# pairlab/SlotFormer

Hardware: AMD Instinct MI355X
Metric: rollout frames/sec at B=32, 128x128, 7 slots, 6+50 steps (SAVi-encode + SlotFormer rollout) (higher is better)
Workload: dtype f32 storage; matmul/conv on split-bf16 MFMA (bf16x3: hi*hi+hi*lo+lo*hi, f32 accumulate)

## Files before the change

include/slotformer_hip.h:

```cpp
#ifndef SLOTFORMER_HIP_H
#define SLOTFORMER_HIP_H
#include <stddef.h>

#ifdef __cplusplus
extern "C" {
#endif

int sf_version(void);
const char* sf_last_error_string(void);

int sf_get_precision(void);
int sf_set_precision(int mode);

int sf_profile_enable(int class_mask);
int sf_set_seam_fused(int on);
int sf_get_seam_fused(void);
int sf_set_ffn_rows64(int on);
int sf_get_ffn_rows64(void);
int sf_profile_sample(int every);
int sf_profile_read(int kernel_class, double* total_ms, long long* launches, double* work);


int sf_linear_f32(const float* A, int lda, const float* W, const float* bias, const float* ln_gamma,
                  const float* ln_beta, float ln_eps, const float* residual, int ldr, float* C, int ldc,
                  int M, int N, int K, int relu, void* stream);

int sf_layernorm_f32(const float* x, const float* gamma, const float* beta, float* y, int rows, int D,
                     float eps, void* stream);

int sf_conv2d_nchw_in_f32(const float* img, long long frame_stride, const float* weight, const float* bias,
                          const float* add, float* out, int F, int Cin, int Hin, int Win, int Cout, int ks,
                          int stride, int relu, void* stream);
int sf_conv2d_nchw_in_grouped_f32(const float* img, long long frame_stride, int fgroup, long long group_stride, const float* weight,
                                  const float* bias, const float* add, float* out, int F, int Cin, int Hin, int Win, int Cout, int ks,
                                  int stride, int relu, void* stream);

int sf_conv2d_nhwc_f32(const float* in, const float* w_packed, const float* bias, const float* add, float* out,
                       int F, int H, int W, int Cin, int Cout, int ks, int relu, void* stream);
int sf_pack_conv_weight_f32(const float* w_oihw, float* w_ohwi, int Cout, int Cin, int ks, void* stream);
int sf_pixel_feat_f32(const float* x, const float* ln0_g, const float* ln0_b, const float* w1, const float* b1, const float* w2,
                      const float* b2, const float* ln1_g, const float* ln1_b, float* feat, int M, float eps, int form, void* stream);
size_t sf_conv_frag_bytes(int Cout, int Cin, int ks);
int sf_set_conv_fp16x2(int on);
int sf_get_conv_fp16x2(void);
int sf_pack_conv_frag_weights(const float* w_ohwi, void* frag, int Cout, int Cin, int ks, void* stream);
int sf_conv5x5_frag_f32(const float* in, const void* w_frag, const float* bias, const float* add, float* out, int F, int H, int W,
                        int relu, void* stream);
int sf_conv5x5_ws_f32(const float* in, const void* w_frag, const float* bias, const float* add, float* out, int F, int H, int W,
                      int relu, int n_workgroups, void* stream);

size_t sf_deconv_frag_bytes(int Cout, int Cin, int ks, int stride);
int sf_pack_deconv_frag_weights(const float* w_ohwi, void* frag, int Cout, int Cin, int ks, int stride, void* stream);
int sf_deconv5x5s2_frag_f32(const float* in, const void* w_frag, const float* bias, float* out, int R, int H, int W, int relu, void* stream);
int sf_deconv5x5s2_head_frag_f32(const float* in, const void* w_frag, const float* bias, const float* head_w, const float* head_b, float* dec,
                                 int R, int H, int W, void* stream);
int sf_decode_l0_expand_f32(const float* table, const float* posterm, float* out, int R, int res, int C1, void* stream);

int sf_conv_transpose2d_nhwc_f32(const float* in, const float* w_packed, const float* bias, float* out, int F,
                                 int Hin, int Win, int Cin, int Cout, int ks, int stride, int relu, void* stream);
int sf_pack_deconv_weight_f32(const float* w_iohw, float* w_ohwi, int Cin, int Cout, int ks, void* stream);
int sf_slot_broadcast_f32(const float* slots, const float* table, float* out, int R, int P, int D, void* stream);
int sf_decode_combine_f32(const float* dec, float* recon_combined, float* recons, float* masks, int F, int N, int HW,
                          void* stream);
int sf_decode_combine_seg_f32(const float* dec, float* recon_combined, float* recons, float* masks, long long* seg_i64,
                              unsigned char* seg_u8, float fg_thre, unsigned* slot_max, int F, int N, int HW, void* stream);
int sf_postproc_mask_f32(const float* masks, long long* seg_i64, unsigned char* seg_u8, float fg_thre, unsigned* slot_max, int F, int N,
                         int HW, void* stream);

size_t sf_vp_metrics_workspace_bytes(int F, int H, int W);
int sf_vp_image_metrics_f32(const float* gt, const float* pred, double* mse, double* psnr, double* ssim, int F, int H, int W, int to_rgb,
                            void* workspace, size_t workspace_bytes, void* stream);
int sf_vp_mask_metrics(const long long* gt_mask, const void* pred_mask, int pred_is_u8, unsigned* tables, float* pred_boxes, double* ari,
                       double* fari, double* miou, unsigned* flag, int F, int H, int W, int num_classes, void* workspace, size_t workspace_bytes,
                       void* stream);
int sf_vp_bbox_pr_f32(const float* gt_bbox, const unsigned char* gt_pres_mask, const float* pred_bbox, double* ap, double* ar, int F, int N, int M,
                      float ovthresh, void* stream);
int sf_masks_to_boxes(const void* masks, int is_u8, float* boxes, unsigned* flag, int F, int H, int W, int num_boxes, void* stream);
int sf_vp_mean_over_videos_f64(const double* per_video, double* out, int K, int B, int T, void* stream);

typedef struct {
  const void* conv_w[13];
  const float* conv_b[13];
  const float* lin_w[5];
  const float* shift;
  const float* scale;
} sf_lpips_model;
int sf_lpips_pack_conv_weights(const float* w_oihw, void* packed, int Cout, int Cin, void* stream);
int sf_lpips_pack_conv_weights_host(const float* w_oihw, void* packed, int Cout, int Cin);
size_t sf_lpips_workspace_bytes(int H, int W, int chunk);
int sf_lpips_f32(const sf_lpips_model* m, const float* x, const float* y, float* out, int F, int H, int W, int chunk, int normalize,
                 void* workspace, size_t workspace_bytes, void* stream);
int sf_lpips_mean_over_videos_f32(const float* scores, double* per_video, double* mean, int B, int T, void* stream);

size_t sf_ingest_tables_bytes(int H0, int W0, int H, int W, int mode);
int sf_ingest_tables_host(void* tables, size_t bytes, int H0, int W0, int H, int W, int mode);
int sf_ingest_frames_u8(const unsigned char* src, const unsigned char* palette, int K, const void* tables, const float* mean3,
                        const float* std3, float* out, int F, int H0, int W0, int H, int W, int antialias, int max_blocks, void* stream);
int sf_resize_masks_nearest(const void* src, int src_is_u8, const void* tables, long long* out_i64, unsigned char* out_u8, int F, int H0,
                            int W0, int H, int W, void* stream);

int sf_rle_label_maps(const unsigned* run_ends, const int* object_offsets, const int* frame_offsets, const void* tables, long long* labels_i64,
                      unsigned char* labels_u8, int* extents, int F, int num_objects, int num_runs, int h, int w, int H, int W, void* stream);
int sf_rle_boxes_pad(const int* extents, float* bbox, unsigned char* pres_mask, unsigned* flag, int F, int num, void* stream);

enum { SF_EGRESS_TRUNC = 0, SF_EGRESS_NEAREST_EVEN = 1 };
enum { SF_EGRESS_F32_CHW = 0, SF_EGRESS_U8_CHW = 1, SF_EGRESS_U8_HWC = 2 };
enum { SF_EGRESS_IMG = 0, SF_EGRESS_SLOTS = 1, SF_EGRESS_IDS = 2 };
int sf_egress_frames_u8(const float* x, unsigned char* out, long long F, int H, int W, int hwc, int to_rgb, int rounding, void* stream);
typedef struct {
  int kind;
  int N;
  const void* a;
  const void* b;
  float scale;
  int ids_i64;
  int P;
  int history_len;
} sf_egress_tile;
int sf_egress_grid_shape(int K, int H, int W, int nrow, int padding, int border, int* CH, int* CW);
int sf_egress_grid(const sf_egress_tile* tiles, int n_entries, void* out, int out_mode, int T, int H, int W, int nrow, int padding,
                   float pad_value, int border, void* stream);
int sf_egress_draw_boxes(unsigned char* frames, const float* boxes, const unsigned char* pres, const unsigned char* palette, int P, int F, int M,
                         int H, int W, int width, void* stream);

// ... 392 lines not shown
typedef struct {
  int num_slots, slot_size, T, text_len, question_len;
  int d_model, num_heads, ffn_dim, num_layers;
  int vocab, emb_dim;
  int mlp_hidden, num_answers;
  const float* cls;
  const float* pos;
  const float *vision_w, *vision_b;
  const float* q_embedding;
  const float *q_in_proj_w, *q_in_proj_b;
  const sf_tfm_layer* layers;
  const float *cls_w1, *cls_b1, *cls_w2, *cls_b2;
  const float *mc_w1, *mc_b1, *mc_w2, *mc_b2;
} sf_aloe_model;

typedef struct {
  float *cls, *pos, *vision_w, *vision_b, *q_embedding, *q_in_proj_w, *q_in_proj_b;
  const sf_tfm_layer_grads* layers;
  float *cls_w1, *cls_b1, *cls_w2, *cls_b2;
  float *mc_w1, *mc_b1, *mc_w2, *mc_b2;
} sf_aloe_grads;

int sf_aloe_train_ok(int num_slots, int slot_size, int T, int text_len, int d_model, int num_heads, int ffn, int num_layers);
size_t sf_aloe_train_workspace_bytes(const sf_aloe_model* m, int B);
int sf_aloe_train_fwd_f32(const sf_aloe_model* m, const float* slots, long long stride_v, long long stride_t, int V, int T_all, const int* video_index,
                          const int* start, int frame_offset, const int* tokens, const unsigned char* pad_mask, int B1, int Bn, float dropout_p,
                          unsigned long long seed, float* cls_logits, float* mc_logits, unsigned char* gates, unsigned char* head_gates, void* ws,
                          size_t ws_bytes, void* stream);
int sf_aloe_train_bwd_f32(const sf_aloe_model* m, const float* slots, long long stride_v, long long stride_t, int V, int T_all, const int* video_index,
                          const int* start, int frame_offset, const int* tokens, const unsigned char* pad_mask, int B1, int Bn, const float* g_cls,
                          const float* g_mc, const sf_aloe_grads* grads, float dropout_p, unsigned long long seed, void* ws, size_t ws_bytes, void* stream);
int sf_aloe_score_grad_f32(const float* cls_logits, const int* cls_labels, int B1, int num_answers, const float* mc_logits, const float* mc_labels, int Bn,
                           float w_cls, float w_mc, float* losses, float* g_cls, float* g_mc, void* stream);

int sf_rollout_train_clips_fwd_f32(const sf_rollouter* m, const float* table, int T_total, const int* clip_video, const int* clip_start,
                                   int frame_offset, float* pred, int B, int pred_len, float dropout_p, unsigned long long seed, void* ws,
                                   size_t ws_bytes, void* stream);
size_t sf_clip_mse_workspace_bytes(int B, int S, long long E);
int sf_clip_mse_f32(const float* pred, const float* target, const int* clip_video, const int* clip_start, int T_total, int first_frame,
                    int frame_step, const float* step_w, const int* clip_len, int hist, float scale, float* d_pred, double* stats, int B, int S,
                    long long E, void* ws, size_t ws_bytes, void* stream);
int sf_clip_frames_f32(const unsigned char* table, int T_total, const int* clip_video, const int* clip_start, int first_frame, int frame_step,
                       const float* mean3, const float* std3, float* out, int B, int S, int H, int W, void* stream);

int sf_normal_noise_f32(float* out, long long n, unsigned long long seed, unsigned tag, void* stream);
size_t sf_kernel_sample_workspace_bytes(long long R, int D);
int sf_kernel_sample_fwd_f32(const float* dist, const float* noise, unsigned long long seed, unsigned tag, float prior_log_var, float* kernels,
                             double* kld_sum, long long R, int D, void* ws, size_t ws_bytes, void* stream);
int sf_kernel_sample_bwd_f32(const float* dist, const float* noise, unsigned long long seed, unsigned tag, float prior_log_var,
                             const float* d_kernels, const float* d_kld, float kld_scale, float* d_dist, long long R, int D, void* stream);

typedef struct {
  int resolution;
  int enc_layers;
  int enc_channels[9];
  int enc_ks;
  int enc_out_channels, num_slots, slot_size, slot_mlp_size, num_iterations;
  const float* conv_w[8];
  const float* conv_b[8];
  const float* pos_table;
  const float *enc_ln_g, *enc_ln_b, *enc_fc1_w, *enc_fc1_b, *enc_fc2_w, *enc_fc2_b;
  const float *sa_norm_in_g, *sa_norm_in_b, *sa_q_ln_g, *sa_q_ln_b, *sa_q_w;
  const float* sa_kv_w;
  const float *gru_w_ih, *gru_w_hh, *gru_b_ih, *gru_b_hh;
  const float *mlp_ln_g, *mlp_ln_b, *mlp_w1, *mlp_b1, *mlp_w2, *mlp_b2;
  const float* init_latents;
  int kd_mode;
  const float *kd_w0, *kd_b0, *kd_ln_g, *kd_ln_b, *kd_w3, *kd_b3;
  int pred_type;
  int pred_rnn, pred_norm_first, pred_num_layers, pred_num_heads, pred_ffn_dim, pred_hidden;
  const float *pm_ln_g, *pm_ln_b, *pm_w0, *pm_b0, *pm_w2, *pm_b2;
  const sf_tfm_layer* pred_layers;
  const float *lstm_w_ih, *lstm_w_hh, *lstm_b_ih, *lstm_b_hh, *proj_w, *proj_b;
  float sa_eps;
  const float* sa_q_w_t;
  const float *pm_w0_t, *pm_w2_t, *kd_w0_t;
  const void *sa_gru_ih_p, *sa_gru_hh_p, *sa_mlp_w1_p, *sa_mlp_w2_p, *sa_q_w_p;
  const float *sa_fold_q_w, *sa_fold_q_w_t, *sa_fold_gru_ih_t;
  const void *sa_fold_q_w_p, *sa_fold_gru_ih_p;
  const void** pred_packed;
  const void *enc_fc1_p, *enc_fc2_p;
  const void* conv_w_frag[8];
  const void *pm_w0_p, *pm_w2_p, *kd_w0_p;
} sf_savi_encoder;

size_t sf_savi_encode_workspace_bytes(const sf_savi_encoder* m, int B);
int sf_savi_encode_f32(const sf_savi_encoder* m, const float* img, const float* noise, const float* prev_slots,
                       float* lstm_h, float* lstm_c, int state_valid, float* post_slots, float* kernel_dist,
                       float* attn, int B, int T, void* ws, size_t ws_bytes, void* stream);

size_t sf_savi_cnn_workspace_bytes(const sf_savi_encoder* m, int B);
int sf_savi_cnn_f32(const sf_savi_encoder* m, const float* img, int B, int T, int t0, int t1, float* feat, void* ws,
                    size_t ws_bytes, void* stream);
int sf_savi_encode_pre_f32(const sf_savi_encoder* m, const float* img, const float* feat_pre, int n_pre, const float* noise,
                           const float* prev_slots, float* lstm_h, float* lstm_c, int state_valid, float* post_slots,
                           float* kernel_dist, float* attn, int B, int T, void* ws, size_t ws_bytes, void* stream);
size_t sf_savi_encode_fork_workspace_bytes(const sf_savi_encoder* m, int B, int T);
size_t sf_savi_encode_batched_workspace_bytes(const sf_savi_encoder* m, int B, int T);
int sf_set_encode_fuse_next(int on);
int sf_get_encode_fuse_next(void);
int sf_set_slot_chain(int on);
int sf_get_slot_chain(void);
int sf_set_slot_attn_planes(int on);
int sf_get_slot_attn_planes(void);
int sf_set_pixel_tok(int on);
int sf_get_pixel_tok(void);
int sf_savi_chain_ok(const sf_savi_encoder* m, int B, int T);
size_t sf_savi_planes_bytes(const sf_savi_encoder* m, int B, int T);
size_t sf_savi_features_workspace_bytes(const sf_savi_encoder* m, int B, int T);
int sf_savi_features_planes_f32(const sf_savi_encoder* m, const float* img, int B, int T, void* planes, void* ws, size_t ws_bytes, void* stream);
size_t sf_savi_slots_chain_workspace_bytes(const sf_savi_encoder* m, int videos);
int sf_savi_slots_chain_f32(const sf_savi_encoder* m, const void* planes, const float* noise, const float* prev_slots, float* post, long long post_bs,
                            float* kernel_dist, float* attn, int NB, int B, int T, void* ws, size_t ws_bytes, void* stream);
int sf_savi_encode_fork_f32(const sf_savi_encoder* m, const float* img, const float* feat_pre, int n_pre, const float* noise,
                            const float* prev_slots, float* lstm_h, float* lstm_c, int state_valid, float* post_slots,
                            float* kernel_dist, float* attn, int B, int T, void* ws, size_t ws_bytes, void* stream, void* side_stream);

typedef struct {
  int resolution;
  int dec_layers;
  int dec_channels[9];
  int dec_strides[8];
  int dec_ks, dec_res;
  int num_slots, slot_size;
  const float* deconv_w[8];
  const float* deconv_b[8];
  const float *out_w, *out_b;
  const float* pos_table;
  const float* deconv_w_flipped[8];
  const void* deconv_w_frag[8];
  const float* l0_weff;
  const float* l0_posterm;
} sf_savi_decoder;

size_t sf_savi_decode_workspace_bytes(const sf_savi_decoder* m, int F);
int sf_savi_decode_f32(const sf_savi_decoder* m, const float* slots, float* recon_combined, float* recons,
                       float* masks, int F, void* ws, size_t ws_bytes, void* stream);
int sf_savi_decode_seg_f32(const sf_savi_decoder* m, const float* slots, float* recon_combined, float* recons, float* masks,
                           long long* seg_i64, unsigned char* seg_u8, float fg_thre, int F, void* ws, size_t ws_bytes, void* stream);

typedef struct {
  float* deconv_w[8];
  float* deconv_b[8];
  float *out_w, *out_b, *pos_w, *pos_b;
} sf_savi_decoder_grads;

size_t sf_savi_decode_train_workspace_bytes(const sf_savi_decoder* m, int F);
int sf_savi_decode_train_fwd_f32(const sf_savi_decoder* m, const float* slots, float* recon_combined, float* recons,
                                 float* masks, int F, void* ws, size_t ws_bytes, void* stream);
int sf_savi_decode_train_bwd_f32(const sf_savi_decoder* m, const float* const* deconv_w_bwd, const float* d_recon,
                                 float* d_slots, const float* pos_grid, const sf_savi_decoder_grads* g, int F, void* ws,
                                 size_t ws_bytes, void* stream);

size_t sf_conv_wgrad_partial_floats(int CA, int ks);
int sf_conv_wgrad_f32(const float* A, int CA, int F, int H, int W, const float* X, int Hx, int Wx, int s, int ks, long long rows, float* dW,
                      float* partial, size_t partial_floats, void* stream);
int sf_conv2d_nhwc_bwd_data_f32(const float* in, const float* w_packed, const float* relu_mask, float* out, int F, int Hin, int Win, int Cin,
                                int Cout, int ks, int stride, void* stream);
int sf_pack_conv_bwd_weight_f32(const float* w_oihw, float* w_bwd, int Cout, int Cin, int ks, void* stream);
size_t sf_conv_first_wgrad_workspace_bytes(int F);
int sf_conv_first_wgrad_f32(const float* img, long long frame_stride, int resolution, const float* dY, int F, float* dW, void* ws,
                            size_t ws_bytes, void* stream);
int sf_pos_dense_grad_f32(const float* d, int F, int HW, int C, const float* grid, float* dw, float* db, float* dtab, void* stream);
size_t sf_savi_decode_head_bwd_workspace_bytes(int Cl);
int sf_savi_decode_head_bwd_f32(const float* dec, const float* d_recon, const float* act, const float* out_w, float* d_dec, float* d_act,
                                float* d_out_w, float* d_out_b, int F, int N, int HW, int Cl, void* ws, size_t ws_bytes, void* stream);
// ... 51 lines not shown
```

slotformer_amd/_lib.py:

```python
import ctypes as C
import os

_HERE = os.path.dirname(os.path.abspath(__file__))
LIB_PATH = os.environ.get('SF_LIB_PATH') or os.path.join(_HERE, 'libslotformer_hip.so')

FP = C.c_void_p


class sf_tfm_layer(C.Structure):
    _fields_ = [(n, FP) for n in (
        'norm1_g', 'norm1_b', 'in_proj_w', 'in_proj_b', 'out_proj_w', 'out_proj_b',
        'norm2_g', 'norm2_b', 'lin1_w', 'lin1_b', 'lin2_w', 'lin2_b', 'lin1_packed', 'lin2_packed', 'attn_in_packed', 'attn_out_packed', 'tok_packed')]


class sf_rollouter(C.Structure):
    _fields_ = [(n, C.c_int) for n in (
        'num_slots', 'slot_size', 'd_model', 'num_layers', 'num_heads', 'ffn_dim', 'norm_first',
        'window_len', 'single_step')] + [(n, FP) for n in (
            'in_proj_w', 'in_proj_b', 'out_proj_w', 'out_proj_b', 'pe_tok')] + [
                ('layers', C.POINTER(sf_tfm_layer)), ('in_proj_packed', C.c_void_p), ('out_proj_packed', C.c_void_p)]


class sf_aloe(C.Structure):
    _fields_ = [(n, C.c_int) for n in ('num_slots', 'slot_size', 'T', 'text_len', 'question_len', 'd_model', 'num_heads', 'ffn_dim', 'num_layers',
# ... 16 lines not shown
        (n, FP) for n in ('in_proj_w', 'in_proj_b', 'enc_t_pe', 'cls')] + [('layers', C.POINTER(sf_tfm_layer))] + [
            (n, FP) for n in ('mlp_w1', 'mlp_b1', 'mlp_w2', 'mlp_b2')]


class sf_phyre_readout_grads(C.Structure):
    _fields_ = [(n, FP) for n in ('in_proj_w', 'in_proj_b', 'enc_t_pe', 'cls')] + [('layers', C.POINTER(sf_tfm_layer_grads))] + [
        (n, FP) for n in ('mlp_w1', 'mlp_b1', 'mlp_w2', 'mlp_b2')]


_ALOE_HEADS = ('cls_w1', 'cls_b1', 'cls_w2', 'cls_b2', 'mc_w1', 'mc_b1', 'mc_w2', 'mc_b2')
_ALOE_LEAVES = ('cls', 'pos', 'vision_w', 'vision_b', 'q_embedding', 'q_in_proj_w', 'q_in_proj_b')


class sf_aloe_model(C.Structure):
    _fields_ = [(n, C.c_int) for n in ('num_slots', 'slot_size', 'T', 'text_len', 'question_len', 'd_model', 'num_heads', 'ffn_dim', 'num_layers',
                                       'vocab', 'emb_dim', 'mlp_hidden', 'num_answers')] + [(n, FP) for n in _ALOE_LEAVES] + [
                                           ('layers', C.POINTER(sf_tfm_layer))] + [(n, FP) for n in _ALOE_HEADS]


class sf_aloe_grads(C.Structure):
    _fields_ = [(n, FP) for n in _ALOE_LEAVES] + [('layers', C.POINTER(sf_tfm_layer_grads))] + [(n, FP) for n in _ALOE_HEADS]


class sf_rollouter_grads(C.Structure):
    _fields_ = [(n, FP) for n in ('in_proj_w', 'in_proj_b', 'out_proj_w', 'out_proj_b')] + [
        ('layers', C.POINTER(sf_tfm_layer_grads)), ('pe_tok', FP)]


_SA_LEAVES = ('norm_in_g', 'norm_in_b', 'wk', 'wv', 'q_ln_g', 'q_ln_b', 'wq', 'gru_w_ih', 'gru_w_hh', 'gru_b_ih', 'gru_b_hh',
              'mlp_ln_g', 'mlp_ln_b', 'mlp_w1', 'mlp_b1', 'mlp_w2', 'mlp_b2')


class sf_slot_attention(C.Structure):
    _fields_ = [(n, C.c_int) for n in ('in_features', 'slot_size', 'mlp_hidden', 'num_slots')] + [
        (n, FP) for n in _SA_LEAVES] + [('eps', C.c_float)]


class sf_slot_attention_grads(C.Structure):
    _fields_ = [(n, FP) for n in _SA_LEAVES]


class sf_adam_group(C.Structure):
    _fields_ = [('begin', C.c_longlong), ('lr', C.c_float)]


class sf_savi_decoder_grads(C.Structure):
    _fields_ = [('deconv_w', FP * 8), ('deconv_b', FP * 8)] + [(n, FP) for n in ('out_w', 'out_b', 'pos_w', 'pos_b')]


class sf_savi_features(C.Structure):
    _fields_ = [(n, C.c_int) for n in ('resolution', 'layers', 'channels', 'ks', 'hidden', 'out_channels')] + [
        ('conv_w', FP * 8), ('conv_b', FP * 8)] + [(n, FP) for n in ('pos_grid', 'pos_w', 'pos_b', 'ln_g', 'ln_b', 'fc1_w', 'fc1_b',
                                                                      'fc2_w', 'fc2_b')]


class sf_savi_features_grads(C.Structure):
    _fields_ = [('conv_w', FP * 8), ('conv_b', FP * 8)] + [(n, FP) for n in ('pos_w', 'pos_b', 'ln_g', 'ln_b', 'fc1_w', 'fc1_b',
                                                                              'fc2_w', 'fc2_b')]


class sf_savi_encoder(C.Structure):
    _fields_ = (
        [('resolution', C.c_int), ('enc_layers', C.c_int), ('enc_channels', C.c_int * 9),
         ('enc_ks', C.c_int)] +
        [(n, C.c_int) for n in ('enc_out_channels', 'num_slots', 'slot_size', 'slot_mlp_size',
                                'num_iterations')] +
        [('conv_w', FP * 8), ('conv_b', FP * 8), ('pos_table', FP)] +
        [(n, FP) for n in ('enc_ln_g', 'enc_ln_b', 'enc_fc1_w', 'enc_fc1_b', 'enc_fc2_w', 'enc_fc2_b',
                           'sa_norm_in_g', 'sa_norm_in_b', 'sa_q_ln_g', 'sa_q_ln_b', 'sa_q_w', 'sa_kv_w',
                           'gru_w_ih', 'gru_w_hh', 'gru_b_ih', 'gru_b_hh',
                           'mlp_ln_g', 'mlp_ln_b', 'mlp_w1', 'mlp_b1', 'mlp_w2', 'mlp_b2',
                           'init_latents')] +
        [('kd_mode', C.c_int)] +
        [(n, FP) for n in ('kd_w0', 'kd_b0', 'kd_ln_g', 'kd_ln_b', 'kd_w3', 'kd_b3')] +
        [(n, C.c_int) for n in ('pred_type', 'pred_rnn', 'pred_norm_first', 'pred_num_layers',
                                'pred_num_heads', 'pred_ffn_dim', 'pred_hidden')] +
        [(n, FP) for n in ('pm_ln_g', 'pm_ln_b', 'pm_w0', 'pm_b0', 'pm_w2', 'pm_b2')] +
        [('pred_layers', C.POINTER(sf_tfm_layer))] +
        [(n, FP) for n in ('lstm_w_ih', 'lstm_w_hh', 'lstm_b_ih', 'lstm_b_hh', 'proj_w', 'proj_b')] +
        [('sa_eps', C.c_float), ('sa_q_w_t', FP), ('pm_w0_t', FP), ('pm_w2_t', FP), ('kd_w0_t', FP),
         ('sa_gru_ih_p', C.c_void_p), ('sa_gru_hh_p', C.c_void_p), ('sa_mlp_w1_p', C.c_void_p), ('sa_mlp_w2_p', C.c_void_p),
         ('sa_q_w_p', C.c_void_p), ('sa_fold_q_w', FP), ('sa_fold_q_w_t', FP), ('sa_fold_gru_ih_t', FP), ('sa_fold_q_w_p', C.c_void_p),
         ('sa_fold_gru_ih_p', C.c_void_p), ('pred_packed', C.POINTER(C.c_void_p)), ('enc_fc1_p', C.c_void_p), ('enc_fc2_p', C.c_void_p),
         ('conv_w_frag', C.c_void_p * 8), ('pm_w0_p', C.c_void_p), ('pm_w2_p', C.c_void_p), ('kd_w0_p', C.c_void_p)])


class sf_slate_block(C.Structure):
    _fields_ = [(n, FP) for n in ('ln1_g', 'ln1_b', 'wqkv', 'wo', 'ln2_g', 'ln2_b', 'wq_c', 'wkv_c', 'wo_c', 'ln3_g', 'ln3_b',
                                  'w1', 'b1', 'w2', 'b2')] + [('is_first', C.c_int)]


class sf_slate_decoder(C.Structure):
    _fields_ = [(n, C.c_int) for n in ('d_model', 'num_heads', 'num_layers', 'vocab_size', 'num_slots', 'max_len')] + [
        (n, FP) for n in ('in_proj_w', 'in_proj_b', 'tok_emb', 'pos_emb', 'lnf_g', 'lnf_b', 'head_w')] + [
            ('blocks', C.POINTER(sf_slate_block))]


class sf_slate_step_opts(C.Structure):
    _fields_ = [('soft_rows', FP), ('conv0_t', FP), ('conv0_width', C.c_int), ('soft_scale', C.c_float), ('soft_seed', C.c_ulonglong),
                ('sample', C.c_int), ('inv_temperature', C.c_float), ('sample_seed', C.c_ulonglong), ('row_base', C.c_longlong)]


class sf_savi_decoder(C.Structure):
    _fields_ = ([('resolution', C.c_int), ('dec_layers', C.c_int), ('dec_channels', C.c_int * 9),
                 ('dec_strides', C.c_int * 8), ('dec_ks', C.c_int), ('dec_res', C.c_int), ('num_slots', C.c_int),
                 ('slot_size', C.c_int), ('deconv_w', FP * 8), ('deconv_b', FP * 8), ('out_w', FP), ('out_b', FP),
                 ('pos_table', FP), ('deconv_w_flipped', FP * 8), ('deconv_w_frag', C.c_void_p * 8), ('l0_weff', FP), ('l0_posterm', FP)])


class sf_egress_tile(C.Structure):
    _fields_ = [('kind', C.c_int), ('N', C.c_int), ('a', C.c_void_p), ('b', C.c_void_p), ('scale', C.c_float), ('ids_i64', C.c_int), ('P', C.c_int),
                ('history_len', C.c_int)]


class sf_lpips_model(C.Structure):
    _fields_ = [('conv_w', C.c_void_p * 13), ('conv_b', FP * 13), ('lin_w', FP * 5), ('shift', FP), ('scale', FP)]


I, LL, F32, SZ, VP = C.c_int, C.c_longlong, C.c_float, C.c_size_t, C.c_void_p

SIGNATURES = {
    'sf_version': (I, []),
    'sf_last_error_string': (C.c_char_p, []),
    'sf_get_precision': (I, []),
    'sf_set_precision': (I, [I]),
    'sf_profile_enable': (I, [I]),
    'sf_profile_sample': (I, [I]),
    'sf_set_seam_fused': (I, [I]),
    'sf_get_seam_fused': (I, []),
    'sf_set_ffn_rows64': (I, [I]),
    'sf_get_ffn_rows64': (I, []),
    'sf_profile_read': (I, [I, C.POINTER(C.c_double), C.POINTER(C.c_longlong), C.POINTER(C.c_double)]),
    'sf_linear_f32': (I, [FP, I, FP, FP, FP, FP, F32, FP, I, FP, I, I, I, I, I, VP]),
    'sf_layernorm_f32': (I, [FP, FP, FP, FP, I, I, F32, VP]),
    'sf_conv2d_nchw_in_f32': (I, [FP, LL, FP, FP, FP, FP, I, I, I, I, I, I, I, I, VP]),
    'sf_conv2d_nchw_in_grouped_f32': (I, [FP, LL, I, LL, FP, FP, FP, FP, I, I, I, I, I, I, I, I, VP]),
    'sf_conv2d_nhwc_f32': (I, [FP, FP, FP, FP, FP, I, I, I, I, I, I, I, VP]),
    'sf_pack_conv_weight_f32': (I, [FP, FP, I, I, I, VP]),
    'sf_pixel_feat_f32': (I, [FP] * 10 + [I, F32, I, VP]),
    'sf_conv_frag_bytes': (SZ, [I, I, I]),
    'sf_set_conv_fp16x2': (I, [I]),
    'sf_get_conv_fp16x2': (I, []),
    'sf_pack_conv_frag_weights': (I, [FP, VP, I, I, I, VP]),
    'sf_conv5x5_frag_f32': (I, [FP, VP, FP, FP, FP, I, I, I, I, VP]),
    'sf_conv5x5_ws_f32': (I, [FP, VP, FP, FP, FP, I, I, I, I, I, VP]),
    'sf_deconv_frag_bytes': (SZ, [I, I, I, I]),
    'sf_pack_deconv_frag_weights': (I, [FP, VP, I, I, I, I, VP]),
    'sf_deconv5x5s2_frag_f32': (I, [FP, VP, FP, FP, I, I, I, I, VP]),
    'sf_deconv5x5s2_head_frag_f32': (I, [FP, VP, FP, FP, FP, FP, I, I, I, VP]),
    'sf_decode_l0_expand_f32': (I, [FP, FP, FP, I, I, I, VP]),
    'sf_conv_transpose2d_nhwc_f32': (I, [FP, FP, FP, FP, I, I, I, I, I, I, I, I, VP]),
    'sf_pack_deconv_weight_f32': (I, [FP, FP, I, I, I, VP]),
    'sf_slot_broadcast_f32': (I, [FP, FP, FP, I, I, I, VP]),
    'sf_decode_combine_f32': (I, [FP, FP, FP, FP, I, I, I, VP]),
    'sf_savi_decode_workspace_bytes': (SZ, [C.POINTER(sf_savi_decoder), I]),
    'sf_savi_decode_f32': (I, [C.POINTER(sf_savi_decoder), FP, FP, FP, FP, I, VP, SZ, VP]),
    'sf_savi_decode_seg_f32': (I, [C.POINTER(sf_savi_decoder), FP, FP, FP, FP, VP, VP, F32, I, VP, SZ, VP]),
    'sf_decode_combine_seg_f32': (I, [FP, FP, FP, FP, VP, VP, F32, VP, I, I, I, VP]),
    'sf_postproc_mask_f32': (I, [FP, VP, VP, F32, VP, I, I, I, VP]),
    'sf_vp_metrics_workspace_bytes': (SZ, [I, I, I]),
    'sf_vp_image_metrics_f32': (I, [FP, FP, VP, VP, VP, I, I, I, I, VP, SZ, VP]),
    'sf_vp_mask_metrics': (I, [VP, VP, I, VP, FP, VP, VP, VP, VP, I, I, I, I, VP, SZ, VP]),
    'sf_vp_bbox_pr_f32': (I, [FP, VP, FP, VP, VP, I, I, I, F32, VP]),
    'sf_masks_to_boxes': (I, [VP, I, FP, VP, I, I, I, I, VP]),
    'sf_vp_mean_over_videos_f64': (I, [VP, VP, I, I, I, VP]),
    'sf_lpips_pack_conv_weights': (I, [FP, VP, I, I, VP]),
    'sf_lpips_pack_conv_weights_host': (I, [VP, VP, I, I]),
    'sf_lpips_workspace_bytes': (SZ, [I, I, I]),
    'sf_lpips_f32': (I, [C.POINTER(sf_lpips_model), FP, FP, FP, I, I, I, I, I, VP, SZ, VP]),
    'sf_lpips_mean_over_videos_f32': (I, [FP, VP, VP, I, I, VP]),
    'sf_ingest_tables_bytes': (SZ, [I, I, I, I, I]),
    'sf_ingest_tables_host': (I, [VP, SZ, I, I, I, I, I]),
    'sf_ingest_frames_u8': (I, [VP, VP, I, VP, FP, FP, FP, I, I, I, I, I, I, I, VP]),
    'sf_resize_masks_nearest': (I, [VP, I, VP, VP, VP, I, I, I, I, I, VP]),
    'sf_rle_label_maps': (I, [VP, VP, VP, VP, VP, VP, VP, I, I, I, I, I, I, I, VP]),
    'sf_rle_boxes_pad': (I, [VP, FP, VP, VP, I, I, VP]),
    'sf_egress_frames_u8': (I, [FP, VP, LL, I, I, I, I, I, VP]),
    'sf_egress_grid_shape': (I, [I, I, I, I, I, I, C.POINTER(I), C.POINTER(I)]),
    'sf_egress_grid': (I, [C.POINTER(sf_egress_tile), I, VP, I, I, I, I, I, I, F32, I, VP]),
    'sf_egress_draw_boxes': (I, [VP, FP, VP, VP, I, I, I, I, I, I, VP]),
    'sf_pos_embed_table_f32': (I, [FP, FP, FP, FP, I, I, VP]),
    'sf_slot_attn_num_partials': (I, [I]),
    'sf_slot_attn_iter_f32': (I, [FP, FP, I, LL, FP, FP, FP, FP, I, I, I, I, F32, F32, VP]),
    'sf_slot_update_f32': (I, [FP, FP, I, FP] + [FP] * 10 + [FP, I, I, I, I, F32, VP]),
    'sf_slot_update_packed_f32': (I, [FP, FP, I, FP, VP, VP, FP, FP, FP, FP, VP, FP, VP, FP, FP, FP, FP, VP, FP, I, I, I, I, F32, VP]),
    'sf_slot_attn_iter_planes_f32': (I, [VP, LL, FP, FP, FP, FP, LL, I, I, I, F32, F32, VP]),
    'sf_slot_prologue_f32': (I, [FP] * 8 + [I, FP, FP, FP, LL, FP, LL, FP, FP, FP, FP, FP, I, I, I, F32, VP]),
    'sf_slot_update_packed_next_f32': (I, [FP, FP, I, FP, VP, VP, FP, FP, FP, FP, VP, FP, VP, FP, FP, FP, FP, VP, FP, I, I, I, I, F32,
                                           FP, LL, I, FP, FP, VP, FP, VP, FP, I, VP, FP, FP, LL, FP, LL, FP, VP]),
    'sf_mha_f32': (I, [FP, FP, I, I, I, I, I, VP]),
    'sf_qkv_attention_f32': (I, [FP, FP, FP, F32, FP, FP, FP, I, I, I, I, I, VP]),
    'sf_lstm_pointwise_f32': (I, [FP, FP, FP, FP, I, I, VP]),
    'sf_sample_dist_f32': (I, [FP, FP, FP, I, I, VP]),
    'sf_bilinear_resize_f32': (I, [FP, FP, LL, I, I, I, I, VP]),
    'sf_rollout_workspace_bytes': (SZ, [C.POINTER(sf_rollouter), I]),
    'sf_rollout_f32': (I, [C.POINTER(sf_rollouter), FP, I, I, I, VP, SZ, VP]),
    'sf_rollout_opts_f32': (I, [C.POINTER(sf_rollouter), FP, I, I, I, VP, SZ, VP, C.POINTER(sf_rollout_opts)]),
    'sf_rollout_phases_workspace_bytes': (SZ, [C.POINTER(sf_rollouter), I, I]),
    'sf_rollout_phases_f32': (I, [C.POINTER(sf_rollouter), FP, I, I, I, I, I, VP, SZ, VP, C.POINTER(sf_rollout_opts)]),
    'sf_rollout_uses_seam': (I, [C.POINTER(sf_rollouter), I]),
    'sf_rollout_uses_seam_opts': (I, [C.POINTER(sf_rollouter), I, C.POINTER(sf_rollout_opts)]),
    'sf_rollout_is_fused': (I, [C.POINTER(sf_rollouter)]),
    'sf_rollout_tok_ok': (I, [C.POINTER(sf_rollouter)]),
    'sf_rollout_tok_layers': (I, [C.POINTER(sf_rollouter), I, C.POINTER(sf_rollout_opts)]),
    'sf_ffn_chunk_partials_f32': (I, [C.POINTER(sf_tfm_layer), FP, LL, FP, LL, I, I, I, VP]),
    'sf_attn_block_f32': (I, [C.POINTER(sf_tfm_layer), FP, FP, I, I, I, I, VP]),
    'sf_ffn_block_rows_f32': (I, [C.POINTER(sf_tfm_layer), FP, FP, I, I, VP]),
    'sf_set_layer_tok': (I, [I]),
    'sf_get_layer_tok': (I, []),
    'sf_layer_tok_packed_bytes': (SZ, []),
    'sf_layer_tok_packed_bytes_ex': (SZ, [I, I, I]),
    'sf_pack_layer_tok_weights': (I, [C.POINTER(sf_tfm_layer), VP, I, I, I, VP]),
    'sf_layer_tok_block_f32': (I, [C.POINTER(sf_tfm_layer), I, FP, FP, I, I, VP]),
    'sf_layer_tok_block_ex_f32': (I, [C.POINTER(sf_tfm_layer), I, I, I, I, FP, FP, I, I, VP]),
    'sf_debug_read_ts_layer_tok': (I, [C.POINTER(C.c_longlong)]),
    'sf_attn_rows_planes_bytes': (SZ, [I]),
    'sf_attn_block_rows_f32': (I, [C.POINTER(sf_tfm_layer), FP, FP, VP, I, I, I, VP]),
    'sf_slot_attn_iter_bwd_workspace_bytes': (SZ, [I, I, I, I]),
    'sf_slot_attn_iter_bwd_f32': (I, [FP, FP, I, LL, FP, FP, FP, I, FP, FP, FP, I, FP, I, I, I, I, F32, F32, VP, SZ, VP]),
    'sf_slot_attn_iter_bwd16_workspace_bytes': (SZ, [I, I, I, I]),
    'sf_slot_attn_iter_bwd16_f32': (I, [FP, FP, I, LL, FP, FP, FP, I, FP, FP, FP, I, FP, I, I, I, I, F32, F32, VP, SZ, VP]),
    'sf_set_slot_attn_tile16': (I, [I]),
# ... 268 lines not shown
```

slotformer_amd/csrc/engine.hip:

```cpp
#include "../../include/slotformer_hip.h"
#include "sf_internal.h"
#include "sf_arena.h"
#include <map>
#include <vector>
#include "layer_fused.h"
#include "slot_chain.h"
#include <stdlib.h>

namespace {

inline bool plain_gemms(const SfThreadOpts& o) { return o.precision == 2 || o.precision == 3; }

struct TfmWs {
  float *x2, *qkv, *att, *hid, *y;
};

bool tfm_ws_take(SfArena& bp, TfmWs& w, int M, int d, int ffn) {
  w.x2 = bp.take((size_t)M * d);
  w.qkv = bp.take((size_t)M * 3 * d);
  w.att = bp.take((size_t)M * d);
  w.hid = bp.take((size_t)M * ffn);
  w.y = bp.take((size_t)M * d);
  return bp.ok;
}
// ... 434 lines not shown
}

size_t sf_rollout_phases_workspace_bytes(const sf_rollouter* m, int B, int frame_offset) {
  if (!m || B <= 0 || frame_offset <= 0 || (long long)B * frame_offset > 0x7fffffffLL) return 0;
  return sf_rollout_workspace_bytes(m, B * frame_offset);
}

int sf_rollout_phases_f32(const sf_rollouter* m, float* slots, int B, int T_total, int obs, int frame_offset, int pred_len, void* ws,
                          size_t ws_bytes, void* stream, const sf_rollout_opts* opts) {
  SF_REQUIRE(m && slots && ws, "null pointer");
  SF_REQUIRE(B >= 1 && pred_len >= 0, "bad batch / pred_len");
  SF_REQUIRE(frame_offset >= 1, "sf_rollout_phases_f32: frame_offset >= 1");
  SF_REQUIRE(!(m->single_step && frame_offset > 1), "sf_rollout_phases_f32: a single-step rollouter takes frame_offset 1 only");
  SF_REQUIRE(m->window_len >= 1, "bad rollouter shape");
  const int f = frame_offset, hist = m->single_step ? 1 : m->window_len;
  SF_REQUIRE((long long)obs >= (long long)hist * f, "sf_rollout_phases_f32: fewer observed frames than burn-in * frame_offset");
  const long long S = ((long long)pred_len + f - 1) / f;
  SF_REQUIRE((long long)T_total >= obs + S * f, "slots buffer shorter than obs + ceil(pred_len / frame_offset) * frame_offset");
  const int first = obs - hist * f;
  if (!opts) return rollout_run(m, slots, B, T_total, first, f, (int)S, ws, ws_bytes, stream);
  SF_TRY(check_rollout_opts(opts));
  OptsScope scope(rollout_thread_opts(opts));
  return rollout_run(m, slots, B, T_total, first, f, (int)S, ws, ws_bytes, stream);
}

int sf_rollout_is_fused(const sf_rollouter* m) { return plan_rollout(m, 1, sf_thread_opts()).fused(); }

int sf_rollout_tok_ok(const sf_rollouter* m) {
  SfThreadOpts o = sf_thread_opts();
  o.layer_tok = 1;
  const RolloutPlan p = plan_rollout(m, 1, o);
  return p.fused() && p.tok_layers > 0;
}

int sf_rollout_tok_layers(const sf_rollouter* m, int B, const sf_rollout_opts* opts) {
  if (B <= 0) return 0;
  return plan_rollout(m, B, rollout_thread_opts(opts)).tok_layers;
}

int sf_rollout_uses_seam_opts(const sf_rollouter* m, int B, const sf_rollout_opts* opts) {
  if (B <= 0 || !plan_rollout(m, B, rollout_thread_opts(opts)).seam) return 0;
  for (int s = 1; s <= m->window_len; ++s) {
    int nf, f0;
    step_window(m, s, nf, f0);
    if (sf_seam_window_ok(nf * m->num_slots, m->num_slots)) return 1;
  }
  return 0;
}
int sf_rollout_uses_seam(const sf_rollouter* m, int B) { return sf_rollout_uses_seam_opts(m, B, nullptr); }

int sf_rollout_bf16(const sf_rollouter* m, float* slots, int B, int T_total, int pred_len, void* ws, size_t ws_bytes,
                    void* stream) {
  sf_rollout_opts o = {2, -1, 0, 0};
  return sf_rollout_opts_f32(m, slots, B, T_total, pred_len, ws, ws_bytes, stream, &o);
}

}

namespace {
int enc_chunk(int B) { return B < 32 ? B : 32; }
constexpr int ENC_FORK_AHEAD = 4;
int enc_fork_steps(int T) { return T < 2 ? 2 : (T < ENC_FORK_AHEAD ? T : ENC_FORK_AHEAD); }
constexpr int ENC_HW = 64 * 64;

int enc_cmax(const sf_savi_encoder* m) {
  int cmax = 0;
  for (int i = 1; i <= m->enc_layers && i < 9; ++i) cmax = m->enc_channels[i] > cmax ? m->enc_channels[i] : cmax;
  return cmax;
}
void enc_cnn_take(SfArena& bp, float** buf, int n, const sf_savi_encoder* m, size_t frames) {
  for (int i = 0; i < n; ++i) buf[i] = bp.take(frames * ENC_HW * enc_cmax(m));
}

struct SlotRows { float *a, *b, *lat, *q; };
void slot_rows_take(SfArena& bp, SlotRows& r, size_t rows, int D) {
  for (float** f : {&r.a, &r.b, &r.lat, &r.q}) *f = bp.take(rows * D);
}

struct EncodePlan {
  bool fork = false;
  int KV = 2;
  int n_pre = 0;
  bool batched = false;
  enum Feat { KV_GEMMS, KV_FUSED, FOLD_ROWS, FOLD_192, FOLD_PLANES } feat = KV_GEMMS;
  const float *q_w = nullptr, *q_w_t = nullptr, *gru_ih_t = nullptr;
  const void *q_w_p = nullptr, *gru_ih_p = nullptr;
  enum Update { VALU, WIDE, MFMA } update = VALU;
  int p_step = 1;
  bool pred_step = false;
  bool prologue = false;
  bool fuse_next = false;
  bool chain_model = false;
  bool chain = false;
  bool fold() const { return feat >= FOLD_ROWS; }
};

struct EncodeWs {
  float* feat[2];
  float *h1, *h2;
  float* kv;
  SlotRows rows;
  float *lnbuf, *px;
  float *kdist, *kdtmp;
  float *pnum, *pden;
  TfmWs tw;
  float* gates;
  float* big[3];
  float* planes;
};

bool enc_ws_take(SfArena& bp, EncodeWs& w, const sf_savi_encoder* m, int B, int T, const EncodePlan& p) {
  const int N = m->num_slots, D = m->slot_size, Ce = m->enc_out_channels, P = sf_sa_pick_partials(ENC_HW);
  const size_t R = (size_t)B * N, Bc = enc_chunk(B), HW = ENC_HW;
  enc_cnn_take(bp, w.feat, 2, m, Bc);
  w.h1 = bp.take(Bc * HW * Ce);
  w.h2 = bp.take(Bc * HW * Ce);
  w.kv = bp.take((size_t)p.KV * B * HW * 2 * D);
  slot_rows_take(bp, w.rows, R, D);
  w.lnbuf = bp.take(R * D);
  w.px = bp.take(R * D);
  w.kdist = bp.take(R * 2 * D);
  w.kdtmp = bp.take(R * 2 * D);
  w.pnum = bp.take((size_t)B * P * N * D);
  w.pden = bp.take((size_t)B * P * N);
  tfm_ws_take(bp, w.tw, (int)R, D, m->pred_ffn_dim > 2 * D ? m->pred_ffn_dim : 2 * D);
  w.gates = bp.take(R * 4 * (m->pred_hidden > 0 ? m->pred_hidden : 1));
  if (p.batched) enc_cnn_take(bp, w.big, 3, m, (size_t)B * T);
  if (p.chain) w.planes = bp.take((size_t)B * T * HW * 128);
  return bp.ok;
}

size_t enc_ws_bytes(const sf_savi_encoder* m, int B, int T, const EncodePlan& p) {
  SfArena bp(nullptr);
  EncodeWs w;
  enc_ws_take(bp, w, m, B, T, p);
  return bp.bytes() + 8192;
}

bool enc_batched_ok(const sf_savi_encoder* m, int B, int T, int precision) {
  if (T < 2 || B > enc_chunk(B) || (long long)B * T > 384 || m->enc_layers < 2 || precision != 1) return false;
  for (int i = 1; i < m->enc_layers; ++i)
    if (!m->conv_w_frag[i] || m->enc_channels[i] != 64 || m->enc_channels[i + 1] != 64) return false;
  return true;
}

EncodePlan plan_encode(const sf_savi_encoder* m, int B, int T, int n_pre, bool fork, size_t ws_bytes) {
  EncodePlan p;
  p.fork = fork;
  p.KV = fork ? enc_fork_steps(T) : 2;
  p.n_pre = n_pre;
  if (!m || m->enc_layers < 1 || m->enc_layers > 8) return p;
  const int precision = sf_get_precision();
  const int HW = ENC_HW, N = m->num_slots, D = m->slot_size, Ce = m->enc_out_channels, Hm = m->slot_mlp_size, P = sf_sa_pick_partials(HW);
  const int Cl = m->enc_channels[m->enc_layers];
  const bool feat192 = Cl == 64 && Ce == 192 && m->enc_fc1_p && m->enc_fc2_p;
  const bool fold = precision >= 1 && m->sa_fold_q_w && m->sa_fold_q_w_t && m->sa_fold_gru_ih_t && Ce == D && (sf_pixel_mlp_feat_ok(Cl, Ce) || feat192);
  const bool planes = fold && !feat192 && sf_switch(SF_SW_SLOT_ATTN_PLANES) && sf_slot_attn_planes_ok(HW, D, N) && Cl == 64 && P == HW / 256;
  p.feat = fold ? (feat192 ? EncodePlan::FOLD_192 : planes ? EncodePlan::FOLD_PLANES : EncodePlan::FOLD_ROWS)
                : (precision >= 1 ? EncodePlan::KV_FUSED : EncodePlan::KV_GEMMS);
  p.q_w = fold ? m->sa_fold_q_w : m->sa_q_w;
  p.q_w_t = fold ? m->sa_fold_q_w_t : m->sa_q_w_t;
  p.gru_ih_t = fold ? m->sa_fold_gru_ih_t : m->gru_w_ih;
  p.q_w_p = fold ? m->sa_fold_q_w_p : m->sa_q_w_p;
  p.gru_ih_p = fold ? m->sa_fold_gru_ih_p : m->sa_gru_ih_p;
  const bool su_packed = precision >= 1 && p.gru_ih_p && m->sa_gru_hh_p && m->sa_mlp_w1_p && m->sa_mlp_w2_p && p.q_w_p;
  p.update = !su_packed ? EncodePlan::VALU : sf_slot_update_mfma_ok(D, Hm, P) ? EncodePlan::MFMA
            : sf_slot_update_wide_ok(D, Hm, P) ? EncodePlan::WIDE : EncodePlan::VALU;
  if (fold && P == HW / 256 && (planes || sf_slot_attn_sparse_records_n(nullptr, nullptr, HW, D, N))) p.p_step = 2;
  p.pred_step = m->pred_type == 1 && m->pred_packed && precision >= 1;
  p.prologue = m->pred_type == 0 && !m->pred_rnn && m->kd_mode == 1 && m->pm_w0_t && m->pm_w2_t && m->kd_w0_t && p.q_w_t;
  p.fuse_next = p.prologue && p.update == EncodePlan::MFMA && m->pm_w0_p && m->pm_w2_p && m->kd_w0_p && m->pm_ln_g && m->pm_ln_b && m->pm_b0 &&
                m->pm_b2 && m->kd_b0 && sf_switch(SF_SW_ENCODE_FUSE_NEXT);
  p.chain_model = precision == 1 && fold && p.feat != EncodePlan::FOLD_192 && p.update == EncodePlan::MFMA && p.fuse_next &&
                  sf_slot_chain_ok(D, Hm, HW, N) && m->init_latents && m->enc_fc1_w && m->enc_fc2_w;
  p.batched = !fork && n_pre == 0 && enc_batched_ok(m, B, T, precision);
  p.chain = p.batched && p.chain_model && sf_switch(SF_SW_SLOT_CHAIN);
  if (p.chain && ws_bytes < enc_ws_bytes(m, B, T, p)) p.chain = false;
  if (p.batched && ws_bytes < enc_ws_bytes(m, B, T, p)) p.batched = false;
  return p;
}

int run_cnn_layers(const sf_savi_encoder* m, const float* src, long long frame_stride, int nb, float* dst, float* featA, float* featB,
                   int i0, int i1, hipStream_t st) {
  const int res = m->resolution;
  for (int i = i0; i < i1; ++i) {
    const bool lastc = (i == m->enc_layers - 1);
    const int cin = m->enc_channels[i], cout = m->enc_channels[i + 1];
    const float* add = lastc ? m->pos_table : nullptr;
    float* out = lastc ? dst : ((i & 1) ? featB : featA);
    const float* cur = i == 0 ? nullptr : (((i - 1) & 1) ? featB : featA);
    if (i == 0) {
      SF_TRY(sf_conv2d_nchw_in_f32(src, frame_stride, m->conv_w[0], m->conv_b[0], add, out, nb, cin, res, res, cout,
                                   m->enc_ks, res == 128 ? 2 : 1, lastc ? 0 : 1, st));
    } else {
      int rc = 1;
      if (rc == 1 && m->conv_w_frag[i])
        rc = sf_conv5x5_ws_ex(cur, m->conv_w_frag[i], m->conv_b[i], add, out, nb, 64, 64, cin, cout, m->enc_ks, lastc ? 0 : 1, 0, st);
      if (rc == 1 && m->conv_w_frag[i])
        rc = sf_conv5x5_rows4_ex(cur, m->conv_w_frag[i], m->conv_b[i], add, out, nb, 64, 64, cin, cout, m->enc_ks, lastc ? 0 : 1, st);
      if (rc < 0 || rc > 1) return rc;
      if (rc == 1)
        SF_TRY(sf_conv2d_nhwc_f32(cur, m->conv_w[i], m->conv_b[i], add, out, nb, 64, 64, cin, cout, m->enc_ks, lastc ? 0 : 1, st));
    }
  }
  return 0;
}

int enc_cnn_all_steps(const sf_savi_encoder* m, const float* img, int B, int T, float* const* big, hipStream_t st) {
  const int res = m->resolution, c1 = m->enc_channels[1];
  const long long frame_elems = (long long)3 * res * res;
  const int rc = sf_conv_first_grouped_ex(img, (long long)T * frame_elems, B, frame_elems, m->conv_w[0], m->conv_b[0], nullptr, big[0], B * T,
                                          m->enc_channels[0], res, res, c1, m->enc_ks, res == 128 ? 2 : 1, 1, st);
  if (rc < 0 || rc > 1) return rc;
  for (int t = 0; t < T && rc == 1; ++t)
    SF_TRY(sf_conv2d_nchw_in_f32(img + (long long)t * frame_elems, (long long)T * frame_elems, m->conv_w[0], m->conv_b[0], nullptr,
                                 big[0] + (long long)t * B * ENC_HW * c1, B, m->enc_channels[0], res, res, c1, m->enc_ks, res == 128 ? 2 : 1, 1, st));
  return run_cnn_layers(m, nullptr, 0, B * T, big[2], big[0], big[1], 1, m->enc_layers, st);
}

int enc_feature_planes(const sf_savi_encoder* m, const float* img, int B, int T, float* const* big, void* planes, hipStream_t st) {
  SF_TRY(enc_cnn_all_steps(m, img, B, T, big, st));
  return sf_pixel_mlp_feat_planes_ex(big[2], m->enc_ln_g, m->enc_ln_b, m->enc_fc1_w, m->enc_fc1_b, m->enc_fc2_w, m->enc_fc2_b, m->sa_norm_in_g, m->sa_norm_in_b,
                                     planes, B * T * ENC_HW, 1e-5f, st);
}
int enc_slots_chain(const sf_savi_encoder* m, const void* planes, const float* noise, const float* prev, float* post, long long post_bs, float* kernel_dist,
                    float* attn, int NB, int B, int T, const SlotRows& r, hipStream_t st) {
  const int N = m->num_slots, D = m->slot_size;
  const float ln_eps = 1e-5f;
  const int pr = sf_slot_prologue_ex(prev, m->init_latents, m->pm_ln_g, m->pm_ln_b, m->pm_w0_t, m->pm_b0, m->pm_w2_t, m->pm_b2, m->pred_norm_first, m->kd_w0_t,
                                     m->kd_b0, noise, (long long)T * N * D, kernel_dist, (long long)T * N * 2 * D, m->sa_q_ln_g, m->sa_q_ln_b, m->sa_fold_q_w_t,
                                     r.a, r.q, NB * B, N, D, ln_eps, st);
  if (pr != 0) return pr < 0 ? pr : sf_set_err(-1, "the one-launch slot prologue does not apply to this model", __FILE__, __LINE__);
  SfChainWeights cw;
  cw.gru_ih_p = m->sa_fold_gru_ih_p; cw.gru_hh_p = m->sa_gru_hh_p; cw.gru_b_ih = m->gru_b_ih; cw.gru_b_hh = m->gru_b_hh; cw.ln_g = m->mlp_ln_g; cw.ln_b = m->mlp_ln_b;
  cw.w1_p = m->sa_mlp_w1_p; cw.b1 = m->mlp_b1; cw.w2_p = m->sa_mlp_w2_p; cw.b2 = m->mlp_b2; cw.q_ln_g = m->sa_q_ln_g; cw.q_ln_b = m->sa_q_ln_b; cw.q_w_p = m->sa_fold_q_w_p;
  cw.pm_ln_g = m->pm_ln_g; cw.pm_ln_b = m->pm_ln_b; cw.pm_w0_p = m->pm_w0_p; cw.pm_b0 = m->pm_b0; cw.pm_w2_p = m->pm_w2_p; cw.pm_b2 = m->pm_b2;
  cw.pm_norm_first = m->pred_norm_first; cw.kd_w_p = m->kd_w0_p; cw.kd_b = m->kd_b0;
  return sf_slot_chain_ex(planes, NB, B, T, ENC_HW, N, m->num_iterations, 1.0f / sqrtf((float)D), m->sa_eps, ln_eps, r.a, r.b, r.lat, r.q, post, post_bs, attn,
                          noise, kernel_dist, &cw, st);
}

hipEvent_t enc_fork_event(int i) {
  thread_local std::map<int, std::vector<hipEvent_t>> per_dev;
  int dev = 0;
  if (hipGetDevice(&dev) != hipSuccess) return nullptr;
  std::vector<hipEvent_t>& ev = per_dev[dev];
  while ((int)ev.size() <= i) {
    hipEvent_t e = nullptr;
    if (hipEventCreateWithFlags(&e, hipEventDisableTiming) != hipSuccess) return nullptr;
    ev.push_back(e);
  }
  return ev[i];
}
int enc_fork_record(int i, hipStream_t s) {
  const hipEvent_t e = enc_fork_event(i);
  SF_REQUIRE(e != nullptr, "hipEventCreate failed");
  return hipEventRecord(e, s) == hipSuccess ? 0 : sf_set_err((int)hipGetLastError(), "hipEventRecord", __FILE__, __LINE__);
}
int enc_fork_wait(int i, hipStream_t s) {
  return hipStreamWaitEvent(s, enc_fork_event(i), 0) == hipSuccess ? 0 : sf_set_err((int)hipGetLastError(), "hipStreamWaitEvent", __FILE__, __LINE__);
}

struct EncodeArgs {
  const sf_savi_encoder* m;
  const float *img, *feat_pre, *noise;
  float *lstm_h, *lstm_c, *post, *kernel_dist, *attn;
  int B, T;
};

int enc_step_features(const EncodeArgs& a, const EncodePlan& p, const EncodeWs& w, int t, float* kv, hipStream_t st) {
  const sf_savi_encoder* m = a.m;
  const int HW = ENC_HW, B = a.B, Bc = enc_chunk(B), Cl = m->enc_channels[m->enc_layers], Ce = m->enc_out_channels, D = m->slot_size;
  const long long frame_elems = (long long)3 * m->resolution * m->resolution;
  const float ln_eps = 1e-5f;
  for (int b0 = 0; b0 < B; b0 += Bc) {
    const int nb = (B - b0 < Bc) ? (B - b0) : Bc, Mp = nb * HW;
    const float* cur;
    if (t < p.n_pre) {
      cur = a.feat_pre + ((long long)t * B + b0) * HW * Cl;
    } else if (p.batched) {
      cur = w.big[2] + ((long long)t * B + b0) * HW * Cl;
    } else {
      float* dstf = (m->enc_layers & 1) ? w.feat[0] : w.feat[1];
      SF_TRY(run_cnn_layers(m, a.img + ((long long)b0 * a.T + t) * frame_elems, (long long)a.T * frame_elems, nb, dstf, w.feat[0], w.feat[1], 0,
                            m->enc_layers, st));
      cur = dstf;
    }
    if (p.feat == EncodePlan::FOLD_192) {
      SF_TRY(sf_pixel_mlp_feat192_ex(cur, m->enc_ln_g, m->enc_ln_b, m->enc_fc1_p, m->enc_fc1_b, m->enc_fc2_p, m->enc_fc2_b,
                                     m->sa_norm_in_g, m->sa_norm_in_b, kv + (long long)b0 * HW * Ce, Mp, ln_eps, st));
    } else if (p.feat == EncodePlan::FOLD_PLANES) {
      SF_TRY(sf_pixel_mlp_feat_planes_ex(cur, m->enc_ln_g, m->enc_ln_b, m->enc_fc1_w, m->enc_fc1_b, m->enc_fc2_w, m->enc_fc2_b, m->sa_norm_in_g, m->sa_norm_in_b,
                                         (char*)kv + (size_t)b0 * HW * 512, Mp, ln_eps, st));
    } else if (p.feat == EncodePlan::FOLD_ROWS) {
      SF_TRY(sf_pixel_mlp_feat_ex(cur, m->enc_ln_g, m->enc_ln_b, m->enc_fc1_w, m->enc_fc1_b, m->enc_fc2_w, m->enc_fc2_b,
                                  m->sa_norm_in_g, m->sa_norm_in_b, kv + (long long)b0 * HW * Ce, Mp, ln_eps, st));
    } else {
      float* kv_dst = kv + (long long)b0 * HW * 2 * D;
      int rc = 1;
      if (p.feat == EncodePlan::KV_FUSED)
        rc = sf_pixel_mlp_kv_ex(cur, m->enc_ln_g, m->enc_ln_b, m->enc_fc1_w, m->enc_fc1_b, m->enc_fc2_w, m->enc_fc2_b, m->sa_norm_in_g, m->sa_norm_in_b,
                                m->sa_kv_w, kv_dst, Mp, Cl, Ce, 2 * D, ln_eps, st);
      if (rc < 0 || rc > 1) return rc;
      if (rc == 1) {
        SF_TRY(sf_linear_ex(cur, sf_rows(Cl), m->enc_fc1_w, m->enc_fc1_b, m->enc_ln_g, m->enc_ln_b, ln_eps, nullptr,
                            sf_rows(Ce), 0, w.h1, sf_rows(Ce), Mp, Ce, Cl, 1, st));
        SF_TRY(sf_linear_ex(w.h1, sf_rows(Ce), m->enc_fc2_w, m->enc_fc2_b, nullptr, nullptr, ln_eps, nullptr,
                            sf_rows(Ce), 0, w.h2, sf_rows(Ce), Mp, Ce, Ce, 0, st));
        SF_TRY(sf_linear_ex(w.h2, sf_rows(Ce), m->sa_kv_w, nullptr, m->sa_norm_in_g, m->sa_norm_in_b, ln_eps, nullptr,
                            sf_rows(2 * D), 0, kv_dst, sf_rows(2 * D), Mp, 2 * D, Ce, 0, st));
      }
    }
  }
  return 0;
}

int enc_predict(const EncodeArgs& a, const EncodePlan& p, const EncodeWs& w, const float* prev, hipStream_t st, const float** lat) {
  const sf_savi_encoder* m = a.m;
  const int N = m->num_slots, D = m->slot_size, R = a.B * N;
  const float ln_eps = 1e-5f;
  *lat = w.rows.lat;
  if (prev == nullptr) return sf_copy_rows_ex(m->init_latents, sf_rows_batched(D, N, 0, 0), w.rows.lat, sf_rows(D), R, D, st);
  int rc = 1;
  if (p.pred_step)
    rc = sf_pred_step_ex(prev, m->pred_layers, m->pred_num_layers, m->pred_num_heads, m->pred_ffn_dim, m->pred_norm_first, m->pred_packed, m->lstm_b_ih,
                         m->lstm_b_hh, m->proj_b, m->pred_hidden, m->pred_rnn ? a.lstm_h : nullptr, m->pred_rnn ? a.lstm_c : nullptr, w.rows.lat, a.B, N, D,
                         ln_eps, st);
  if (rc != 1) return rc;
  const float* pout;
  if (m->pred_type == 0) {
    SF_TRY(sf_layernorm_ex(prev, sf_rows(D), m->pm_ln_g, m->pm_ln_b, w.lnbuf, sf_rows(D), R, D, ln_eps, st));
    SF_TRY(sf_linear_ex(w.lnbuf, sf_rows(D), m->pm_w0, m->pm_b0, nullptr, nullptr, ln_eps, nullptr, sf_rows(D), 0,
                        w.tw.hid, sf_rows(2 * D), R, 2 * D, D, 1, st));
    SF_TRY(sf_linear_ex(w.tw.hid, sf_rows(2 * D), m->pm_w2, m->pm_b2, nullptr, nullptr, ln_eps,
                        m->pred_norm_first ? w.lnbuf : prev, sf_rows(D), 0, w.px, sf_rows(D), R, D, 2 * D, 0, st));
    pout = w.px;
  } else {
    SF_TRY(sf_copy_rows_ex(prev, sf_rows(D), w.px, sf_rows(D), R, D, st));
    float* cur = w.px;
    TfmWs tw = w.tw;
    for (int l = 0; l < m->pred_num_layers; ++l)
      SF_TRY(tfm_layer(m->pred_layers[l], cur, tw, a.B, N, N, D, m->pred_num_heads, m->pred_ffn_dim, m->pred_norm_first, st, &cur));
    pout = cur;
  }
  *lat = m->pred_rnn ? w.rows.lat : pout;
  if (!m->pred_rnn) return 0;
  const int Hh = m->pred_hidden;
  SF_TRY(sf_linear_ex(pout, sf_rows(D), m->lstm_w_ih, m->lstm_b_ih, nullptr, nullptr, ln_eps, nullptr,
                      sf_rows(4 * Hh), 0, w.gates, sf_rows(4 * Hh), R, 4 * Hh, D, 0, st));
  SF_TRY(sf_linear_ex(a.lstm_h, sf_rows(Hh), m->lstm_w_hh, m->lstm_b_hh, nullptr, nullptr, ln_eps, w.gates,
                      sf_rows(4 * Hh), 0, w.gates, sf_rows(4 * Hh), R, 4 * Hh, Hh, 0, st));
  SF_TRY(sf_lstm_pointwise_ex(w.gates, a.lstm_c, a.lstm_h, a.lstm_c, R, Hh, st));
  return sf_linear_ex(a.lstm_h, sf_rows(Hh), m->proj_w, m->proj_b, nullptr, nullptr, ln_eps, nullptr,
                      sf_rows(D), 0, w.rows.lat, sf_rows(D), R, D, Hh, 0, st);
}

int enc_slot_init(const EncodeArgs& a, const EncodePlan& p, const EncodeWs& w, const float* prev, int t, hipStream_t st, bool* one_launch) {
  const sf_savi_encoder* m = a.m;
  const int N = m->num_slots, D = m->slot_size, R = a.B * N, T = a.T;
  const float ln_eps = 1e-5f;
  int rc = 1;
  if (p.prologue)
    rc = sf_slot_prologue_ex(prev, m->init_latents, m->pm_ln_g, m->pm_ln_b, m->pm_w0_t, m->pm_b0, m->pm_w2_t, m->pm_b2, m->pred_norm_first, m->kd_w0_t,
                             m->kd_b0, a.noise ? a.noise + (long long)t * N * D : nullptr, (long long)T * N * D,
                             a.kernel_dist ? a.kernel_dist + (long long)t * N * 2 * D : nullptr, (long long)T * N * 2 * D, m->sa_q_ln_g, m->sa_q_ln_b,
                             p.q_w_t, w.rows.a, w.rows.q, a.B, N, D, ln_eps, st);
  *one_launch = rc == 0;
  if (rc != 1) return rc;
  const float* lat;
  SF_TRY(enc_predict(a, p, w, prev, st, &lat));
  if (m->kd_mode == 0) {
    SF_TRY(sf_copy_rows_ex(lat, sf_rows(D), w.rows.a, sf_rows(D), R, D, st));
  } else {
    SF_TRY(sf_linear_ex(lat, sf_rows(D), m->kd_w0, m->kd_b0, nullptr, nullptr, ln_eps, nullptr, sf_rows(2 * D), 0,
                        m->kd_mode == 1 ? w.kdist : w.kdtmp, sf_rows(2 * D), R, 2 * D, D, 0, st));
    if (m->kd_mode == 2)
      SF_TRY(sf_linear_ex(w.kdtmp, sf_rows(2 * D), m->kd_w3, m->kd_b3, m->kd_ln_g, m->kd_ln_b, ln_eps, nullptr,
                          sf_rows(2 * D), 0, w.kdist, sf_rows(2 * D), R, 2 * D, 2 * D, 0, st, 1));
    const SfRowMap nmap = sf_rows_batched(D, N, (long long)T * N * D, (long long)t * N * D);
// ... 37 lines not shown
                                    m->sa_mlp_w1_p, m->mlp_b1, m->sa_mlp_w2_p, m->mlp_b2, s_out, post, post_bs, m->sa_q_ln_g, m->sa_q_ln_b,
                                    p.q_w_p, last_it ? nullptr : w.rows.q, B, N, ln_eps, st));
    } else {
      SF_TRY(sf_slot_update_ex(w.pnum, w.pden, P, s_in, p.gru_ih_t, m->gru_w_hh, m->gru_b_ih, m->gru_b_hh, m->mlp_ln_g, m->mlp_ln_b, m->mlp_w1,
                               m->mlp_b1, m->mlp_w2, m->mlp_b2, s_out, post, post_bs, m->sa_q_ln_g, m->sa_q_ln_b, p.q_w_t,
                               (last_it || !p.q_w_t) ? nullptr : w.rows.q, B, N, D, Hm, ln_eps, st));
      if (!last_it && !p.q_w_t)
        SF_TRY(sf_linear_ex(s_out, sf_rows(D), p.q_w, nullptr, m->sa_q_ln_g, m->sa_q_ln_b, ln_eps, nullptr, sf_rows(D), 0, w.rows.q,
                            sf_rows(D), B * N, D, D, 0, st));
    }
    std::swap(s_in, s_out);
  }
  *out = s_in;
  return 0;
}
}

extern "C" {

size_t sf_savi_encode_workspace_bytes(const sf_savi_encoder* m, int B) {
  return (m && B > 0) ? enc_ws_bytes(m, B, 1, plan_encode(m, B, 1, 0, false, 0)) : 0;
}
size_t sf_savi_encode_fork_workspace_bytes(const sf_savi_encoder* m, int B, int T) {
  return (m && B > 0 && T >= 1) ? enc_ws_bytes(m, B, T, plan_encode(m, B, T, 0, true, 0)) : 0;
}
size_t sf_savi_encode_batched_workspace_bytes(const sf_savi_encoder* m, int B, int T) {
  return (m && B > 0 && T > 0) ? enc_ws_bytes(m, B, T, plan_encode(m, B, T, 0, false, ~(size_t)0)) : 0;
}

size_t sf_savi_cnn_workspace_bytes(const sf_savi_encoder* m, int B) {
  if (!m || B <= 0) return 0;
  SfArena bp(nullptr);
  float* feat[2];
  enc_cnn_take(bp, feat, 2, m, enc_chunk(B));
  return bp.bytes() + 4096;
}

int sf_savi_cnn_f32(const sf_savi_encoder* m, const float* img, int B, int T, int t0, int t1, float* feat, void* ws,
                    size_t ws_bytes, void* stream) {
  SF_REQUIRE(m && img && feat && ws, "null pointer");
  SF_REQUIRE(B >= 1 && T >= 1 && t0 >= 0 && t1 >= t0 && t1 <= T, "bad batch / time range");
  SF_REQUIRE(m->resolution == 64 || m->resolution == 128, "resolution must be 64 or 128 (savi.py:226,236)");
  SF_REQUIRE(m->enc_layers >= 1 && m->enc_layers <= 8 && m->pos_table, "bad CNN config");
  SF_REQUIRE(ws_bytes >= sf_savi_cnn_workspace_bytes(m, B), "workspace too small");
  for (int i = 0; i < m->enc_layers; ++i) SF_REQUIRE(m->conv_w[i] != nullptr, "null conv weight");
  const int Bc = enc_chunk(B), HW = ENC_HW, Cl = m->enc_channels[m->enc_layers];
  SfArena bp(ws, ws_bytes);
  float* fb[2];
  enc_cnn_take(bp, fb, 2, m, Bc);
  if (!bp.ok) return sf_set_err(-1, "workspace too small", __FILE__, __LINE__);
  const long long frame_elems = (long long)3 * m->resolution * m->resolution;
  sf_prof_suppress(1);
  int rc = 0;
  for (int t = t0; t < t1 && rc == 0; ++t)
    for (int b0 = 0; b0 < B && rc == 0; b0 += Bc) {
      const int nb = (B - b0 < Bc) ? (B - b0) : Bc;
      rc = run_cnn_layers(m, img + ((long long)b0 * T + t) * frame_elems, (long long)T * frame_elems, nb,
                          feat + ((long long)(t - t0) * B + b0) * HW * Cl, fb[0], fb[1], 0, m->enc_layers, (hipStream_t)stream);
    }
  sf_prof_suppress(0);
  return rc;
}

int sf_savi_chain_ok(const sf_savi_encoder* m, int B, int T) {
  const EncodePlan p = plan_encode(m, B, T, 0, false, ~(size_t)0);
  return (p.batched && p.chain_model) ? 1 : 0;
}
size_t sf_savi_planes_bytes(const sf_savi_encoder* m, int B, int T) { return (m && B > 0 && T > 0) ? (size_t)B * T * ENC_HW * 512 : 0; }
size_t sf_savi_features_workspace_bytes(const sf_savi_encoder* m, int B, int T) {
  if (!m || B <= 0 || T <= 0) return 0;
  SfArena bp(nullptr);
  float* big[3];
  enc_cnn_take(bp, big, 3, m, (size_t)B * T);
  return bp.bytes() + 4096;
}
int sf_savi_features_planes_f32(const sf_savi_encoder* m, const float* img, int B, int T, void* planes, void* ws, size_t ws_bytes, void* stream) {
  SF_REQUIRE(m && img && planes && ws, "sf_savi_features_planes_f32: null pointer");
  SF_REQUIRE(B >= 1 && T >= 1 && sf_savi_chain_ok(m, B, T), "sf_savi_features_planes_f32: the video-stationary slot branch does not apply (sf_savi_chain_ok)");
  SF_REQUIRE(ws_bytes >= sf_savi_features_workspace_bytes(m, B, T), "workspace too small");
  SfArena bp(ws, ws_bytes);
  float* big[3];
  enc_cnn_take(bp, big, 3, m, (size_t)B * T);
  if (!bp.ok) return sf_set_err(-1, "workspace too small", __FILE__, __LINE__);
  return enc_feature_planes(m, img, B, T, big, planes, (hipStream_t)stream);
}
size_t sf_savi_slots_chain_workspace_bytes(const sf_savi_encoder* m, int videos) {
  if (!m || videos <= 0) return 0;
  SfArena bp(nullptr);
  SlotRows r;
  slot_rows_take(bp, r, (size_t)videos * m->num_slots, m->slot_size);
  return bp.bytes() + 4096;
}
int sf_savi_slots_chain_f32(const sf_savi_encoder* m, const void* planes, const float* noise, const float* prev_slots, float* post, long long post_bs,
                            float* kernel_dist, float* attn, int NB, int B, int T, void* ws, size_t ws_bytes, void* stream) {
  SF_REQUIRE(m && planes && post && ws, "sf_savi_slots_chain_f32: null pointer");
  SF_REQUIRE(NB >= 1 && B >= 1 && T >= 1 && plan_encode(m, B, T, 0, false, 0).chain_model,
             "sf_savi_slots_chain_f32: the video-stationary slot branch does not apply (sf_savi_chain_ok)");
  SF_REQUIRE(noise == nullptr || m->kd_mode != 0, "noise given but the model has no kernel_dist layer");
  SF_REQUIRE(ws_bytes >= sf_savi_slots_chain_workspace_bytes(m, NB * B), "workspace too small");
  SfArena bp(ws, ws_bytes);
  SlotRows r;
  slot_rows_take(bp, r, (size_t)NB * B * m->num_slots, m->slot_size);
  if (!bp.ok) return sf_set_err(-1, "workspace too small", __FILE__, __LINE__);
  return enc_slots_chain(m, planes, noise, prev_slots, post, post_bs, kernel_dist, attn, NB, B, T, r, (hipStream_t)stream);
}

int sf_savi_encode_f32(const sf_savi_encoder* m, const float* img, const float* noise, const float* prev_slots,
                       float* lstm_h, float* lstm_c, int state_valid, float* post_slots, float* kernel_dist,
                       float* attn, int B, int T, void* ws, size_t ws_bytes, void* stream) {
  return sf_savi_encode_pre_f32(m, img, nullptr, 0, noise, prev_slots, lstm_h, lstm_c, state_valid, post_slots, kernel_dist,
                                attn, B, T, ws, ws_bytes, stream);
}

int sf_savi_encode_pre_f32(const sf_savi_encoder* m, const float* img, const float* feat_pre, int n_pre, const float* noise,
                           const float* prev_slots, float* lstm_h, float* lstm_c, int state_valid, float* post_slots,
                           float* kernel_dist, float* attn, int B, int T, void* ws, size_t ws_bytes, void* stream) {
  return sf_savi_encode_fork_f32(m, img, feat_pre, n_pre, noise, prev_slots, lstm_h, lstm_c, state_valid, post_slots, kernel_dist, attn,
                                 B, T, ws, ws_bytes, stream, nullptr);
}


int sf_savi_encode_fork_f32(const sf_savi_encoder* m, const float* img, const float* feat_pre, int n_pre, const float* noise,
                            const float* prev_slots, float* lstm_h, float* lstm_c, int state_valid, float* post_slots,
                            float* kernel_dist, float* attn, int B, int T, void* ws, size_t ws_bytes, void* stream, void* side_stream) {
  SF_REQUIRE(m && img && post_slots && ws, "null pointer");
  SF_REQUIRE(n_pre >= 0 && n_pre <= T && (n_pre == 0 || feat_pre != nullptr), "bad precomputed-feature arguments");
  SF_REQUIRE(B >= 1 && T >= 1, "bad batch / clip length");
  SF_REQUIRE(m->resolution == 64 || m->resolution == 128, "resolution must be 64 or 128 (savi.py:226,236)");
  SF_REQUIRE(m->enc_layers >= 1 && m->enc_layers <= 8 && m->enc_channels[0] > 0 && (m->enc_ks & 1), "bad CNN config");
  SF_REQUIRE(m->num_slots >= 1 && m->num_slots <= 16 && m->num_iterations >= 1, "bad slot config (1 <= num_slots <= 16)");
  SF_REQUIRE(m->pos_table && m->enc_ln_g && m->enc_ln_b && m->enc_fc1_w && m->enc_fc1_b && m->enc_fc2_w &&
                 m->enc_fc2_b && m->sa_norm_in_g && m->sa_norm_in_b && m->sa_q_ln_g && m->sa_q_ln_b &&
                 m->sa_q_w && m->sa_kv_w && m->init_latents, "null encoder weight");
  SF_REQUIRE(m->kd_mode >= 0 && m->kd_mode <= 2, "bad kd_mode");
  SF_REQUIRE(m->kd_mode == 0 || (m->kd_w0 && m->kd_b0), "null kernel_dist weight");
  SF_REQUIRE(m->kd_mode != 2 || (m->kd_ln_g && m->kd_ln_b && m->kd_w3 && m->kd_b3), "null kernel_dist weight");
  SF_REQUIRE(noise == nullptr || m->kd_mode != 0, "noise given but the model has no kernel_dist layer");
  if (m->pred_type == 0)
    SF_REQUIRE(m->pm_ln_g && m->pm_ln_b && m->pm_w0 && m->pm_b0 && m->pm_w2 && m->pm_b2, "null predictor weight");
  else
    SF_REQUIRE(check_layers(m->pred_layers, m->pred_num_layers) == 0, "null predictor weight");
  if (m->pred_rnn)
    SF_REQUIRE(lstm_h && lstm_c && m->pred_hidden > 0 && m->lstm_w_ih && m->lstm_w_hh && m->lstm_b_ih &&
                   m->lstm_b_hh && m->proj_w && m->proj_b, "null LSTM state / weight");
  const EncodePlan p = plan_encode(m, B, T, n_pre, side_stream != nullptr && side_stream != stream, ws_bytes);
  for (int i = 0; i < m->enc_layers; ++i) SF_REQUIRE(m->conv_w[i] != nullptr, "null conv weight");
  SfArena bp(ws, ws_bytes);
  EncodeWs w;
  SF_REQUIRE(ws_bytes >= enc_ws_bytes(m, B, T, p) && enc_ws_take(bp, w, m, B, T, p), "workspace too small");
  const hipStream_t st_main = (hipStream_t)stream, st = p.fork ? (hipStream_t)side_stream : st_main;
  const EncodeArgs a{m, img, feat_pre, noise, lstm_h, lstm_c, post_slots, kernel_dist, attn, B, T};
  const int N = m->num_slots, D = m->slot_size;
  const float* prev = prev_slots;
  if (m->pred_rnn && (prev == nullptr || !state_valid)) {
    const long long nz = (long long)B * N * m->pred_hidden;
    hipLaunchKernelGGL(zero_f32_kernel, dim3((unsigned)(((nz + 3) / 4 + 255) / 256)), dim3(256), 0, st_main, lstm_h, lstm_c, nz);
    SF_CHECK_LAUNCH();
  }
  if (p.chain) {
    SF_TRY(enc_feature_planes(m, img, B, T, w.big, w.planes, st_main));
    return enc_slots_chain(m, w.planes, noise, prev, post_slots, (long long)T * N * D, kernel_dist, attn, 1, B, T, w.rows, st_main);
  }
  if (p.batched) SF_TRY(enc_cnn_all_steps(m, img, B, T, w.big, st_main));
  bool next_done = false;
  for (int t = 0; t < T; ++t) {
    float* kv = w.kv + (size_t)(t % p.KV) * B * ENC_HW * 2 * D;
    if (p.fork && t >= p.KV) SF_TRY(enc_fork_wait(T + 1 + (t - p.KV), st_main));
    SF_TRY(enc_step_features(a, p, w, t, kv, st_main));
    if (p.fork) {
      SF_TRY(enc_fork_record(t, st_main));
      SF_TRY(enc_fork_wait(t, st));
    }
    bool one_launch = next_done;
    if (!next_done) SF_TRY(enc_slot_init(a, p, w, prev, t, st, &one_launch));
    next_done = p.fuse_next && one_launch && t + 1 < T;
    SF_TRY(enc_iterations(a, p, w, kv, t, next_done, st, &prev));
    if (p.fork && t + p.KV < T) SF_TRY(enc_fork_record(T + 1 + t, st));
  }
  if (p.fork) {
    SF_TRY(enc_fork_record(T, st));
    SF_TRY(enc_fork_wait(T, st_main));
  }
  return 0;
}

static size_t dec_maxact(const sf_savi_decoder* m) {
  size_t best = (size_t)m->dec_res * m->dec_res * m->dec_channels[0];
  int size = m->dec_res;
  for (int i = 0; i < m->dec_layers && i < 8; ++i) {
    size *= m->dec_strides[i] > 0 ? m->dec_strides[i] : 1;
    const size_t a = (size_t)size * size * m->dec_channels[i + 1];
    best = a > best ? a : best;
  }
  const size_t tab = (size_t)25 * m->dec_channels[1];
  return best > tab ? best : tab;
}
static int dec_chunk(const sf_savi_decoder* m, int F) {
  const double per_frame = (double)m->num_slots * (double)dec_maxact(m);
  int fc = (int)(256.0 * 1024 * 1024 / per_frame);
  if (fc < 1) fc = 1;
  return fc < F ? fc : F;
}

struct DecodeWs {
  float *bufA, *bufB, *dec;
  unsigned* slot_max;
};
static DecodeWs dec_ws_take(SfArena& bp, const sf_savi_decoder* m, int F) {
  const size_t R = (size_t)dec_chunk(m, F) * m->num_slots, HW = (size_t)m->resolution * m->resolution;
  float *a = bp.take(R * dec_maxact(m)), *b = bp.take(R * dec_maxact(m)), *dec = bp.take(R * HW * 4);
  return DecodeWs{a, b, dec, bp.take<unsigned>(R)};
}
size_t sf_savi_decode_workspace_bytes(const sf_savi_decoder* m, int F) {
  if (!m || F <= 0) return 0;
  SfArena bp(nullptr);
  dec_ws_take(bp, m, F);
  return bp.bytes() + 4096;
}

int sf_savi_decode_f32(const sf_savi_decoder* m, const float* slots, float* recon_combined, float* recons,
                       float* masks, int F, void* ws, size_t ws_bytes, void* stream) {
  return sf_savi_decode_seg_f32(m, slots, recon_combined, recons, masks, nullptr, nullptr, 0.5f, F, ws, ws_bytes, stream);
}

int sf_savi_decode_seg_f32(const sf_savi_decoder* m, const float* slots, float* recon_combined, float* recons, float* masks,
                           long long* seg_i64, unsigned char* seg_u8, float fg_thre, int F, void* ws, size_t ws_bytes, void* stream) {
  SF_REQUIRE(m && slots && recon_combined && ws, "null pointer");
  SF_REQUIRE(F >= 1 && m->dec_layers >= 1 && m->dec_layers <= 8 && m->num_slots >= 1 && m->dec_res >= 1 && (m->dec_ks & 1),
             "bad decoder config");
  SF_REQUIRE(m->dec_channels[0] == m->slot_size && (m->slot_size % 4) == 0, "dec_channels[0] must equal slot_size");
  SF_REQUIRE(m->pos_table && m->out_w && m->out_b, "null decoder weight");
  int size = m->dec_res;
  for (int i = 0; i < m->dec_layers; ++i) {
    SF_REQUIRE(m->deconv_w[i] != nullptr && m->dec_strides[i] >= 1 && (m->dec_channels[i + 1] % 4) == 0, "bad deconv layer");
    size *= m->dec_strides[i];
  }
  SF_REQUIRE(size == m->resolution, "decoder output size does not match the resolution (savi.py:279-284)");
  SF_REQUIRE(ws_bytes >= sf_savi_decode_workspace_bytes(m, F), "workspace too small");
  hipStream_t st = (hipStream_t)stream;
  const int N = m->num_slots, D = m->slot_size, res = m->resolution, HW = res * res;
  const int Fc = dec_chunk(m, F);
  SfArena bp(ws, ws_bytes);
  const DecodeWs dw = dec_ws_take(bp, m, F);
  float *bufA = dw.bufA, *bufB = dw.bufB, *dec = dw.dec;
  unsigned* slot_max = dw.slot_max;
  if (!bp.ok) return sf_set_err(-1, "workspace too small", __FILE__, __LINE__);
// ... 58 lines not shown
```

slotformer_amd/csrc/pixel_mlp.hip:

```cpp
#include "sf_internal.h"
#include "slot_chain.h"
#include <stdlib.h>

namespace {
constexpr int PM_NT = 512, PM_ROWS = 128, PM_C0 = 64, PM_C1 = 128, PM_ND = 256;
constexpr int PM_LB0 = PM_C0 + 8, PM_LB1 = PM_C1 + 8;
constexpr int PM_PLANE = PM_ROWS * PM_LB1;
constexpr int PM_H2S = PM_C1 + 4;
constexpr size_t PM_LDS = (size_t)4 * PM_PLANE * sizeof(__bf16) + (2 * PM_ROWS + 4 * PM_C1) * sizeof(float);
static_assert((size_t)PM_ROWS * PM_H2S * 4 <= (size_t)2 * PM_PLANE * 2, "f32 tile must fit in the B planes");
}

template <bool FEAT>
__global__ __launch_bounds__(PM_NT) void pixel_mlp_kv_kernel(
    const float* __restrict__ x, const float* __restrict__ ln0_g, const float* __restrict__ ln0_b,
    const float* __restrict__ w1, const float* __restrict__ b1, const float* __restrict__ w2,
    const float* __restrict__ b2, const float* __restrict__ ln1_g, const float* __restrict__ ln1_b,
    const float* __restrict__ wkv, float* __restrict__ kv, int M, float eps) {
  extern __shared__ __attribute__((aligned(16))) __bf16 lds[];
  __bf16* Ah = lds;
  __bf16* Al = Ah + PM_PLANE;
  __bf16* Bh = Al + PM_PLANE;
  __bf16* Bl = Bh + PM_PLANE;
  float* stats = (float*)(Bl + PM_PLANE);
// ... 113 lines not shown
      *(f32x4*)(H2 + row * PM_H2S + n) = f32x4{acc[j][4 * g] + bv[0], acc[j][4 * g + 1] + bv[1], acc[j][4 * g + 2] + bv[2],
                                             acc[j][4 * g + 3] + bv[3]};
    }
  }
  __syncthreads();

  {
    const int row = t >> 2, part = t & 3;
    f32x4 hv[8];
#pragma unroll
    for (int i = 0; i < 8; ++i) hv[i] = *(const f32x4*)(H2 + row * PM_H2S + part * 32 + 4 * i);
    float s = 0.f;
#pragma unroll
    for (int i = 0; i < 8; ++i) s += (hv[i][0] + hv[i][1]) + (hv[i][2] + hv[i][3]);
    s += sf_dpp<0xB1>(s);
    s += sf_dpp<0x4E>(s);
    const float mean = s * (1.0f / PM_C1);
    float vs = 0.f;
#pragma unroll
    for (int i = 0; i < 8; ++i) {
      const f32x4 dv = hv[i] - mean;
      vs += (dv[0] * dv[0] + dv[1] * dv[1]) + (dv[2] * dv[2] + dv[3] * dv[3]);
    }
    vs += sf_dpp<0xB1>(vs);
    vs += sf_dpp<0x4E>(vs);
    const float rstd = 1.0f / sqrtf(vs * (1.0f / PM_C1) + eps);
#pragma unroll
    for (int i = 0; i < 8; ++i) {
      const int c = part * 32 + 4 * i;
      const f32x4 g = *(const f32x4*)(PV + 2 * PM_C1 + c), be = *(const f32x4*)(PV + 3 * PM_C1 + c);
      if constexpr (FEAT) {
        if (m0 + row < M) *(f32x4*)(kv + (long long)(m0 + row) * PM_C1 + c) = (hv[i] - mean) * rstd * g + be;
      } else {
        bf16x4 hi, lo;
        split4((hv[i] - mean) * rstd * g + be, hi, lo);
        *(bf16x4*)(Ah + row * PM_LB1 + c) = hi;
        *(bf16x4*)(Al + row * PM_LB1 + c) = lo;
      }
    }
  }
  if constexpr (FEAT) return;
  __syncthreads();

#pragma unroll
  for (int half = 0; half < 2; ++half) {
    store_w128(wr3);
    if (half == 0) {
#pragma unroll
      for (int i = 0; i < 8; ++i) wr3[i] = *(const f32x4*)(wkv + (long long)(PM_C1 + q0 + 16 * i) * PM_C1 + 4 * d4);
    }
    __syncthreads();
    gemm(PM_LB1, PM_C1 / 16, acc);
#pragma unroll
    for (int j = 0; j < 2; ++j) {
      const int row = m0 + rb * 32 + (lane & 31);
      if (row < M) {
        float* dst = kv + (long long)row * PM_ND + half * PM_C1 + (cb0 + j) * 32 + 4 * (lane >> 5);
#pragma unroll
        for (int g = 0; g < 4; ++g)
          *(f32x4*)(dst + 8 * g) = f32x4{acc[j][4 * g], acc[j][4 * g + 1], acc[j][4 * g + 2], acc[j][4 * g + 3]};
      }
    }
    __syncthreads();
  }
}

int sf_pixel_mlp_kv_ex(const float* x, const float* ln0_g, const float* ln0_b, const float* w1, const float* b1,
                       const float* w2, const float* b2, const float* ln1_g, const float* ln1_b, const float* wkv,
                       float* kv, int M, int C0, int C1, int ND, float eps, hipStream_t st) {
  if (C0 != PM_C0 || C1 != PM_C1 || ND != PM_ND || M <= 0 || !b1 || !b2) return 1;
  SF_TRY(sf_ensure_dyn_lds((const void*)pixel_mlp_kv_kernel<false>, (size_t)(PM_LDS)));
  static_assert(PM_LDS <= 160 * 1024, "LDS budget");
  sf_prof_begin(SF_K_LINEAR, st, 2.0 * M * (double)(PM_C0 * PM_C1 + PM_C1 * PM_C1 + PM_C1 * PM_ND));
  hipLaunchKernelGGL(pixel_mlp_kv_kernel<false>, dim3((M + PM_ROWS - 1) / PM_ROWS), dim3(PM_NT), PM_LDS, st, x, ln0_g, ln0_b,
                     w1, b1, w2, b2, ln1_g, ln1_b, wkv, kv, M, eps);
  sf_prof_end(SF_K_LINEAR, st);
  SF_CHECK_LAUNCH();
  return 0;
}

bool sf_pixel_mlp_feat_ok(int C0, int C1) { return C0 == PM_C0 && C1 == PM_C1; }
template <bool PLANES>
static int sf_pixel_feat_tok_launch(const float* x, const float* ln0_g, const float* ln0_b, const float* w1, const float* b1, const float* w2, const float* b2,
                                    const float* ln1_g, const float* ln1_b, void* out, int M, float eps, hipStream_t st);

static int sf_pixel_feat_stream_launch(const float* x, const float* ln0_g, const float* ln0_b, const float* w1, const float* b1, const float* w2,
                                       const float* b2, const float* ln1_g, const float* ln1_b, float* feat, int M, float eps, hipStream_t st,
                                       int tile = 0);

int sf_pixel_mlp_feat_ex(const float* x, const float* ln0_g, const float* ln0_b, const float* w1, const float* b1, const float* w2,
                         const float* b2, const float* ln1_g, const float* ln1_b, float* feat, int M, float eps, hipStream_t st) {
  if (M <= 0) return 0;
  constexpr int stream = 1;
  if (sf_switch(SF_SW_PIXEL_TOK)) return sf_pixel_feat_tok_launch<false>(x, ln0_g, ln0_b, w1, b1, w2, b2, ln1_g, ln1_b, feat, M, eps, st);
  if (stream) return sf_pixel_feat_stream_launch(x, ln0_g, ln0_b, w1, b1, w2, b2, ln1_g, ln1_b, feat, M, eps, st);
  SF_TRY(sf_ensure_dyn_lds((const void*)pixel_mlp_kv_kernel<true>, (size_t)(PM_LDS)));
  sf_prof_begin(SF_K_LINEAR, st, 2.0 * M * (double)(PM_C0 * PM_C1 + PM_C1 * PM_C1));
  hipLaunchKernelGGL(pixel_mlp_kv_kernel<true>, dim3((M + PM_ROWS - 1) / PM_ROWS), dim3(PM_NT), PM_LDS, st, x, ln0_g, ln0_b, w1, b1, w2,
                     b2, ln1_g, ln1_b, nullptr, feat, M, eps);
  sf_prof_end(SF_K_LINEAR, st);
  SF_CHECK_LAUNCH();
  return 0;
}

#include "stream_mfma.h"

namespace {
constexpr int PW_NT = 512, PW_ROWS = 128, PW_C0 = 64, PW_C1 = 192, PW_KP = PW_C1 + 8, PW_NB = PW_C1 / 32;
constexpr size_t PW_LDS = (size_t)2 * PW_ROWS * PW_KP * 2 + (size_t)(2 * PW_NB * PW_ROWS + 4 * PW_C1) * 4;
}

__global__ __launch_bounds__(PW_NT) void pixel_mlp_feat192_kernel(const float* __restrict__ x, const float* __restrict__ ln0_g,
                                                                  const float* __restrict__ ln0_b, const uint4* __restrict__ w1p,
                                                                  const float* __restrict__ b1, const uint4* __restrict__ w2p,
                                                                  const float* __restrict__ b2, const float* __restrict__ ln1_g,
                                                                  const float* __restrict__ ln1_b, float* __restrict__ feat, int M, float eps) {
  extern __shared__ __attribute__((aligned(16))) __bf16 pw_lds[];
  __bf16* Ph = pw_lds;
  __bf16* Pl = Ph + PW_ROWS * PW_KP;
  float* S1 = (float*)(Pl + PW_ROWS * PW_KP);
  float* S2 = S1 + PW_NB * PW_ROWS;
  float* PV = S2 + PW_NB * PW_ROWS;
  const int t = threadIdx.x, lane = t & 63, wave = __builtin_amdgcn_readfirstlane(t >> 6);
  const int tok = lane & 31, kg = lane >> 5;
  const int m0 = blockIdx.x * PW_ROWS;
  const int c4 = t & 15, r0 = t >> 4;
  const f32x4 g0 = *(const f32x4*)(ln0_g + 4 * c4), be0 = *(const f32x4*)(ln0_b + 4 * c4);
  float pvv[2];
#pragma unroll
  for (int i = 0; i < 2; ++i) {
    const int j = t + PW_NT * i;
    const float* src = j < PW_C1 ? b1 : j < 2 * PW_C1 ? b2 : j < 3 * PW_C1 ? ln1_g : ln1_b;
    pvv[i] = j < 4 * PW_C1 ? src[j % PW_C1] : 0.f;
  }
  f32x4 xr[4];
#pragma unroll
  for (int i = 0; i < 4; ++i) xr[i] = *(const f32x4*)(x + (long long)min(m0 + r0 + 32 * i, M - 1) * PW_C0 + 4 * c4);
  PsRing<3> s;
  constexpr int KS1 = PW_C0 / 16, KS2 = PW_C1 / 16;
  if (wave < PW_NB) ps_prime<PsChunk<KS1>::CH>(s, w1p, PW_NB, wave, 0, lane);
#pragma unroll
  for (int i = 0; i < 2; ++i)
    if (t + PW_NT * i < 4 * PW_C1) PV[t + PW_NT * i] = pvv[i];
#pragma unroll
  for (int i = 0; i < 4; ++i) {
    const float sm = sf_sum16((xr[i][0] + xr[i][1]) + (xr[i][2] + xr[i][3]));
    const float mean = sm * (1.0f / PW_C0);
    const f32x4 dv = xr[i] - mean;
    const float vs = sf_sum16((dv[0] * dv[0] + dv[1] * dv[1]) + (dv[2] * dv[2] + dv[3] * dv[3]));
    const float rstd = 1.0f / sqrtf(vs * (1.0f / PW_C0) + eps);
    sf_split4(Ph, Pl, (r0 + 32 * i) * PW_KP + 4 * c4, dv * rstd * g0 + be0);
  }
  __syncthreads();
  f32x16 acc[4];
  if (wave < PW_NB) {
#pragma unroll
    for (int rb = 0; rb < 4; ++rb)
#pragma unroll
      for (int r = 0; r < 16; ++r) acc[rb][r] = 0.f;
    ps_blockN<KS1, PsChunk<KS2>::CH, 4>(acc, s, w1p, PW_NB, wave, 0, w2p, PW_NB, wave, 0, Ph, Pl, PW_KP, lane);
  }
  __syncthreads();
  if (wave < PW_NB) {
#pragma unroll
    for (int rb = 0; rb < 4; ++rb)
#pragma unroll
      for (int g = 0; g < 4; ++g) {
        const int n = 32 * wave + 8 * g + 4 * kg;
        const f32x4 bv = *(const f32x4*)(PV + n);
        sf_split4(Ph, Pl, (32 * rb + tok) * PW_KP + n,
                  f32x4{fmaxf(acc[rb][4 * g] + bv[0], 0.f), fmaxf(acc[rb][4 * g + 1] + bv[1], 0.f), fmaxf(acc[rb][4 * g + 2] + bv[2], 0.f),
                        fmaxf(acc[rb][4 * g + 3] + bv[3], 0.f)});
      }
  }
  __syncthreads();
  if (wave < PW_NB) {
#pragma unroll
// ... 218 lines not shown
      for (int g = 0; g < 4; ++g) {
        const int n = cb * 32 + 8 * g + 4 * kg;
        const f32x4 bv = *(const f32x4*)(PV + PM_C1 + n);
        *(f32x4*)(H2 + row * PM_H2S + n) = f32x4{acc[j][4 * g] + bv[0], acc[j][4 * g + 1] + bv[1], acc[j][4 * g + 2] + bv[2],
                                               acc[j][4 * g + 3] + bv[3]};
      }
    }
    __syncthreads();
    {
      const int row = t >> 2, part = t & 3;
      f32x4 hv[8];
#pragma unroll
      for (int i = 0; i < 8; ++i) hv[i] = *(const f32x4*)(H2 + row * PM_H2S + part * 32 + 4 * i);
      float s = 0.f;
#pragma unroll
      for (int i = 0; i < 8; ++i) s += (hv[i][0] + hv[i][1]) + (hv[i][2] + hv[i][3]);
      s += sf_dpp<0xB1>(s);
      s += sf_dpp<0x4E>(s);
      const float mean = s * (1.0f / PM_C1);
      float vs = 0.f;
#pragma unroll
      for (int i = 0; i < 8; ++i) {
        const f32x4 dv = hv[i] - mean;
        vs += (dv[0] * dv[0] + dv[1] * dv[1]) + (dv[2] * dv[2] + dv[3] * dv[3]);
      }
      vs += sf_dpp<0xB1>(vs);
      vs += sf_dpp<0x4E>(vs);
      const float rstd = 1.0f / sqrtf(vs * (1.0f / PM_C1) + eps);
      const int grow = tile * TR + row;
#pragma unroll
      for (int i = 0; i < 8; ++i) {
        const int c = part * 32 + 4 * i;
        const f32x4 g = *(const f32x4*)(PV + 2 * PM_C1 + c), be = *(const f32x4*)(PV + 3 * PM_C1 + c);
        const f32x4 y = (hv[i] - mean) * rstd * g + be;
        if constexpr (PLANES) {
          bf16x4 hi, lo;
          split4(y, hi, lo);
          if (grow < M) {
            __bf16* pr = (__bf16*)feat + (long long)grow * (2 * PM_C1);
            *(bf16x4*)(pr + c) = hi;
            *(bf16x4*)(pr + PM_C1 + c) = lo;
          }
        } else {
          if (grow < M) *(f32x4*)(feat + (long long)grow * PM_C1 + c) = y;
        }
      }
    }
    __syncthreads();
  }
}

template <int TR, bool PLANES = false>
static int sf_pixel_feat_stream_launch_t(const float* x, const float* ln0_g, const float* ln0_b, const float* w1, const float* b1, const float* w2,
                                         const float* b2, const float* ln1_g, const float* ln1_b, float* feat, int M, float eps, hipStream_t st) {
  using Cfg = PfCfg<TR>;
  static_assert(Cfg::LDS <= 160 * 1024, "LDS budget");
  SF_TRY(sf_ensure_dyn_lds((const void*)pixel_feat_stream_kernel<TR, PLANES>, Cfg::LDS));
  const int ntiles = (M + TR - 1) / TR;
  sf_prof_begin(SF_K_LINEAR, st, 2.0 * M * (double)(PM_C0 * PM_C1 + PM_C1 * PM_C1));
  constexpr int env_pix = 0;
  const int tpw = env_pix >= TR ? env_pix / TR : Cfg::TPW;
  hipLaunchKernelGGL((pixel_feat_stream_kernel<TR, PLANES>), dim3((ntiles + tpw - 1) / tpw), dim3(Cfg::NT), Cfg::LDS, st, x, ln0_g, ln0_b, w1, b1,
                     w2, b2, ln1_g, ln1_b, feat, M, eps, tpw);
  sf_prof_end(SF_K_LINEAR, st);
  SF_CHECK_LAUNCH();
  return 0;
}

static int sf_pixel_feat_stream_launch(const float* x, const float* ln0_g, const float* ln0_b, const float* w1, const float* b1, const float* w2,
                                       const float* b2, const float* ln1_g, const float* ln1_b, float* feat, int M, float eps, hipStream_t st,
                                       int tile) {
  if (tile == 0) tile = 64;
  if (tile == 64) return sf_pixel_feat_stream_launch_t<64>(x, ln0_g, ln0_b, w1, b1, w2, b2, ln1_g, ln1_b, feat, M, eps, st);
  return sf_pixel_feat_stream_launch_t<128>(x, ln0_g, ln0_b, w1, b1, w2, b2, ln1_g, ln1_b, feat, M, eps, st);
}

namespace {
constexpr int PT_NT = 512;
constexpr int PT_W1 = 0, PT_W2 = 32 * 1024, PT_VEC = 96 * 1024;
constexpr int PV_G0 = 0, PV_B0 = 64, PV_B1 = 128, PV_B2 = 256, PV_G1 = 384, PV_BE1 = 512, PV_N = 640;
constexpr size_t PT_LDS = (size_t)PT_VEC + PV_N * 4;
}

template <bool PLANES>
__global__ __launch_bounds__(PT_NT) void pixel_feat_tok_kernel(const float* __restrict__ x, const float* __restrict__ ln0_g, const float* __restrict__ ln0_b,
                                                               const float* __restrict__ w1, const float* __restrict__ b1, const float* __restrict__ w2,
                                                               const float* __restrict__ b2, const float* __restrict__ ln1_g, const float* __restrict__ ln1_b,
                                                               void* __restrict__ out, int M, float eps, int tpw) {
  extern __shared__ __attribute__((aligned(16))) char pt_lds[];
  const int t = threadIdx.x, lane = t & 63;
  const int wave = __builtin_amdgcn_readfirstlane(t >> 6);
  const int n = lane & 31, h = lane >> 5;
  {
    f32x4 wa[6], wb[6];
#pragma unroll
    for (int it = 0; it < 6; ++it) {
      const int f = t + it * PT_NT, fl = f & 63, fi = fl & 31, fh = fl >> 5, fr = f >> 6;
      const float* p;
      int second;
      if (fr < 16) {
        const int blk = fr >> 2, ks = fr & 3;
        p = w1 + (long long)(32 * blk + fi) * PM_C0 + 32 * fh + 8 * ks;
        second = 4;
      } else {
        const int g2 = fr - 16, ob = g2 >> 3, blk = (g2 >> 1) & 3, sx = g2 & 1;
        const int orow = 64 * ((fi >> 2) & 1) + 16 * ob + 4 * (fi >> 3) + (fi & 3);
        p = w2 + (long long)orow * PM_C1 + 32 * blk + 16 * sx + 4 * fh;
        second = 8;
      }
      wa[it] = *(const f32x4*)p;
      wb[it] = *(const f32x4*)(p + second);
    }
#pragma unroll
    for (int it = 0; it < 6; ++it) {
      const int f = t + it * PT_NT, fl = f & 63, fr = f >> 6;
      const bf16x4 ah = __builtin_convertvector(wa[it], bf16x4), bh = __builtin_convertvector(wb[it], bf16x4);
      const bf16x4 al = __builtin_convertvector(wa[it] - __builtin_convertvector(ah, f32x4), bf16x4);
      const bf16x4 bl = __builtin_convertvector(wb[it] - __builtin_convertvector(bh, f32x4), bf16x4);
      char* dst = pt_lds + (size_t)fr * 2048 + fl * 16;
      *(bf16x8*)dst = __builtin_shufflevector(ah, bh, 0, 1, 2, 3, 4, 5, 6, 7);
      *(bf16x8*)(dst + 1024) = __builtin_shufflevector(al, bl, 0, 1, 2, 3, 4, 5, 6, 7);
    }
  }
  float* PV = (float*)(pt_lds + PT_VEC);
  for (int i = t; i < PV_N; i += PT_NT)
    PV[i] = i < PV_B0 ? ln0_g[i] : i < PV_B1 ? ln0_b[i - PV_B0] : i < PV_B2 ? b1[i - PV_B1] : i < PV_G1 ? b2[i - PV_B2] : i < PV_BE1 ? ln1_g[i - PV_G1] : ln1_b[i - PV_BE1];
  __syncthreads();
  auto other = [&](float v) {
    const unsigned u = __builtin_bit_cast(unsigned, v);
    const auto r2 = __builtin_amdgcn_permlane32_swap(u, u, false, false);
    return __builtin_bit_cast(float, h ? r2[0] : r2[1]);
  };
  auto pairsum = [&](float v) {
    const float o = other(v);
    return h ? o + v : v + o;
  };
  const char* wl = pt_lds + lane * 16;
  const long long ntile = ((long long)M + 31) / 32, tstep = (long long)gridDim.x * (PT_NT / 64);
  long long tile = (long long)blockIdx.x * (PT_NT / 64) + wave;
  auto row_of = [&](long long tl) {
    const long long px = tl * 32 + n;
    return px < M ? px : (long long)M - 1;
  };
  f32x4 xn[8];
  if (tile < ntile) {
    const float* xr = x + row_of(tile) * PM_C0 + 32 * h;
#pragma unroll
    for (int i = 0; i < 8; ++i) xn[i] = *(const f32x4*)(xr + 4 * i);
  }
#pragma unroll 1
  for (int ti = 0; ti < tpw; ++ti, tile += tstep) {
    if (tile >= ntile) break;
    const long long p0 = tile * 32;
    const long long pix = row_of(tile);
    f32x4 xv[8];
#pragma unroll
    for (int i = 0; i < 8; ++i) xv[i] = xn[i];
    if (tile + tstep < ntile) {
      const float* xr = x + row_of(tile + tstep) * PM_C0 + 32 * h;
#pragma unroll
      for (int i = 0; i < 8; ++i) xn[i] = *(const f32x4*)(xr + 4 * i);
    }
    float s0 = 0.f;
#pragma unroll
    for (int i = 0; i < 8; ++i) s0 += (xv[i][0] + xv[i][1]) + (xv[i][2] + xv[i][3]);
    const float mean = pairsum(s0) * (1.0f / PM_C0);
    float v0 = 0.f;
#pragma unroll
    for (int i = 0; i < 8; ++i) {
      xv[i] -= mean;
      v0 += (xv[i][0] * xv[i][0] + xv[i][1] * xv[i][1]) + (xv[i][2] * xv[i][2] + xv[i][3] * xv[i][3]);
    }
    const float rstd = 1.0f / sqrtf(pairsum(v0) * (1.0f / PM_C0) + eps);
    bf16x8 xh[4], xl[4];
#pragma unroll
    for (int ks = 0; ks < 4; ++ks) {
      const int c = 32 * h + 8 * ks;
      sf_split8(xv[2 * ks] * rstd * *(const f32x4*)(PV + PV_G0 + c) + *(const f32x4*)(PV + PV_B0 + c),
                xv[2 * ks + 1] * rstd * *(const f32x4*)(PV + PV_G0 + c + 4) + *(const f32x4*)(PV + PV_B0 + c + 4), xh[ks], xl[ks]);
    }
    bf16x8 hh[8], hl[8];
#pragma unroll
    for (int bp = 0; bp < 2; ++bp) {
      f32x16 acc[2];
#pragma unroll
      for (int r = 0; r < 16; ++r) acc[0][r] = acc[1][r] = 0.f;
#pragma unroll
      for (int ks = 0; ks < 4; ++ks) {
        bf16x8 wh[2], wlo[2];
#pragma unroll
        for (int e = 0; e < 2; ++e) {
          const char* wp = wl + PT_W1 + ((2 * bp + e) * 4 + ks) * 2048;
          wh[e] = *(const bf16x8*)wp;
          wlo[e] = *(const bf16x8*)(wp + 1024);
        }
        acc[0] = __builtin_amdgcn_mfma_f32_32x32x16_bf16(wh[0], xl[ks], acc[0], 0, 0, 0);
        acc[1] = __builtin_amdgcn_mfma_f32_32x32x16_bf16(wh[1], xl[ks], acc[1], 0, 0, 0);
        acc[0] = __builtin_amdgcn_mfma_f32_32x32x16_bf16(wlo[0], xh[ks], acc[0], 0, 0, 0);
        acc[1] = __builtin_amdgcn_mfma_f32_32x32x16_bf16(wlo[1], xh[ks], acc[1], 0, 0, 0);
        acc[0] = __builtin_amdgcn_mfma_f32_32x32x16_bf16(wh[0], xh[ks], acc[0], 0, 0, 0);
        acc[1] = __builtin_amdgcn_mfma_f32_32x32x16_bf16(wh[1], xh[ks], acc[1], 0, 0, 0);
        __builtin_amdgcn_sched_barrier(0);
      }
#pragma unroll
      for (int e = 0; e < 2; ++e) {
        const int blk = 2 * bp + e;
#pragma unroll
        for (int sx = 0; sx < 2; ++sx) {
          f32x4 u[2];
#pragma unroll
          for (int gg = 0; gg < 2; ++gg) {
            const int g = 2 * sx + gg;
            const f32x4 bb = *(const f32x4*)(PV + PV_B1 + 32 * blk + 8 * g + 4 * h);
#pragma unroll
            for (int q = 0; q < 4; ++q) u[gg][q] = fmaxf(acc[e][4 * g + q] + bb[q], 0.f);
          }
          sf_split8(u[0], u[1], hh[2 * blk + sx], hl[2 * blk + sx]);
        }
      }
    }
    f32x16 Y[4];
#pragma unroll
    for (int op = 0; op < 2; ++op) {
#pragma unroll
      for (int r = 0; r < 16; ++r) Y[2 * op][r] = Y[2 * op + 1][r] = 0.f;
#pragma unroll
      for (int k2 = 0; k2 < 8; ++k2) {
        bf16x8 wh[2], wlo[2];
#pragma unroll
        for (int e = 0; e < 2; ++e) {
          const char* wp = wl + PT_W2 + (((2 * op + e) * 4 + (k2 >> 1)) * 2 + (k2 & 1)) * 2048;
          wh[e] = *(const bf16x8*)wp;
          wlo[e] = *(const bf16x8*)(wp + 1024);
        }
        Y[2 * op] = __builtin_amdgcn_mfma_f32_32x32x16_bf16(wh[0], hl[k2], Y[2 * op], 0, 0, 0);
        Y[2 * op + 1] = __builtin_amdgcn_mfma_f32_32x32x16_bf16(wh[1], hl[k2], Y[2 * op + 1], 0, 0, 0);
        Y[2 * op] = __builtin_amdgcn_mfma_f32_32x32x16_bf16(wlo[0], hh[k2], Y[2 * op], 0, 0, 0);
        Y[2 * op + 1] = __builtin_amdgcn_mfma_f32_32x32x16_bf16(wlo[1], hh[k2], Y[2 * op + 1], 0, 0, 0);
        Y[2 * op] = __builtin_amdgcn_mfma_f32_32x32x16_bf16(wh[0], hh[k2], Y[2 * op], 0, 0, 0);
        Y[2 * op + 1] = __builtin_amdgcn_mfma_f32_32x32x16_bf16(wh[1], hh[k2], Y[2 * op + 1], 0, 0, 0);
        __builtin_amdgcn_sched_barrier(0);
      }
    }
    float s1 = 0.f;
#pragma unroll
    for (int ob = 0; ob < 4; ++ob)
#pragma unroll
      for (int g = 0; g < 4; ++g) {
        const f32x4 bb = *(const f32x4*)(PV + PV_B2 + 64 * h + 16 * ob + 4 * g);
#pragma unroll
        for (int q = 0; q < 4; ++q) {
          Y[ob][4 * g + q] += bb[q];
          s1 += Y[ob][4 * g + q];
        }
      }
    const float mean1 = pairsum(s1) * (1.0f / PM_C1);
    float v1 = 0.f;
#pragma unroll
    for (int ob = 0; ob < 4; ++ob)
#pragma unroll
      for (int r = 0; r < 16; ++r) {
        Y[ob][r] -= mean1;
        v1 += Y[ob][r] * Y[ob][r];
      }
    const float rstd1 = 1.0f / sqrtf(pairsum(v1) * (1.0f / PM_C1) + eps);
    const bool live = p0 + n < M;
#pragma unroll
    for (int ob = 0; ob < 4; ++ob)
#pragma unroll
      for (int gp = 0; gp < 2; ++gp) {
        f32x4 y[2];
#pragma unroll
        for (int gg = 0; gg < 2; ++gg) {
          const int g = 2 * gp + gg, c = 64 * h + 16 * ob + 4 * g;
          const f32x4 ga = *(const f32x4*)(PV + PV_G1 + c), be = *(const f32x4*)(PV + PV_BE1 + c);
#pragma unroll
          for (int q = 0; q < 4; ++q) y[gg][q] = Y[ob][4 * g + q] * rstd1 * ga[q] + be[q];
        }
        const int c0 = 64 * h + 16 * ob + 8 * gp;
        if (live) {
          if constexpr (PLANES) {
            bf16x8 yh, yl;
            sf_split8(y[0], y[1], yh, yl);
            __bf16* pr = (__bf16*)out + pix * (2 * PM_C1);
            *(bf16x8*)(pr + c0) = yh;
            *(bf16x8*)(pr + PM_C1 + c0) = yl;
          } else {
            float* pr = (float*)out + pix * PM_C1;
            *(f32x4*)(pr + c0) = y[0];
            *(f32x4*)(pr + c0 + 4) = y[1];
          }
        }
      }
  }
}

template <bool PLANES>
static int sf_pixel_feat_tok_launch(const float* x, const float* ln0_g, const float* ln0_b, const float* w1, const float* b1, const float* w2, const float* b2,
                                    const float* ln1_g, const float* ln1_b, void* out, int M, float eps, hipStream_t st) {
  static_assert(PT_LDS <= 160 * 1024, "LDS budget");
  SF_TRY(sf_ensure_dyn_lds((const void*)pixel_feat_tok_kernel<PLANES>, PT_LDS));
  const long long ntile = ((long long)M + 31) / 32;
  long long grid = (ntile + (PT_NT / 64) - 1) / (PT_NT / 64);
  const int cus = sf_stream_cus((void*)st);
  if (grid > cus) grid = cus;
  const int tpw = (int)((ntile + grid * (PT_NT / 64) - 1) / (grid * (PT_NT / 64)));
  sf_prof_begin(SF_K_LINEAR, st, 2.0 * M * (double)(PM_C0 * PM_C1 + PM_C1 * PM_C1));
  hipLaunchKernelGGL(pixel_feat_tok_kernel<PLANES>, dim3((unsigned)grid), dim3(PT_NT), PT_LDS, st, x, ln0_g, ln0_b, w1, b1, w2, b2, ln1_g, ln1_b, out, M, eps, tpw);
  sf_prof_end(SF_K_LINEAR, st);
  SF_CHECK_LAUNCH();
  return 0;
}

int sf_pixel_mlp_feat_planes_ex(const float* x, const float* ln0_g, const float* ln0_b, const float* w1, const float* b1, const float* w2,
                                const float* b2, const float* ln1_g, const float* ln1_b, void* planes, int M, float eps, hipStream_t st) {
  if (sf_switch(SF_SW_PIXEL_TOK)) return sf_pixel_feat_tok_launch<true>(x, ln0_g, ln0_b, w1, b1, w2, b2, ln1_g, ln1_b, planes, M, eps, st);
  return sf_pixel_feat_stream_launch_t<64, true>(x, ln0_g, ln0_b, w1, b1, w2, b2, ln1_g, ln1_b, (float*)planes, M, eps, st);
}

extern "C" int sf_pixel_feat_f32(const float* x, const float* ln0_g, const float* ln0_b, const float* w1, const float* b1, const float* w2,
                                 const float* b2, const float* ln1_g, const float* ln1_b, float* feat, int M, float eps, int form, void* stream) {
  SF_REQUIRE(x && ln0_g && ln0_b && w1 && b1 && w2 && b2 && ln1_g && ln1_b && feat && M > 0, "sf_pixel_feat_f32: null pointer / empty problem");
  SF_REQUIRE(form >= 0 && form <= 4, "sf_pixel_feat_f32: form must be 0 .. 4");
  SF_REQUIRE(sf_get_precision() == 1, "sf_pixel_feat_f32: split-bf16 mode only");
  hipStream_t st = (hipStream_t)stream;
  if (form == 4) return sf_pixel_mlp_feat_planes_ex(x, ln0_g, ln0_b, w1, b1, w2, b2, ln1_g, ln1_b, feat, M, eps, st);
  if (form == 3) return sf_pixel_feat_tok_launch<false>(x, ln0_g, ln0_b, w1, b1, w2, b2, ln1_g, ln1_b, feat, M, eps, st);
  if (form >= 1) return sf_pixel_feat_stream_launch(x, ln0_g, ln0_b, w1, b1, w2, b2, ln1_g, ln1_b, feat, M, eps, st, form == 1 ? 128 : 64);
  SF_TRY(sf_ensure_dyn_lds((const void*)pixel_mlp_kv_kernel<true>, (size_t)(PM_LDS)));
  hipLaunchKernelGGL(pixel_mlp_kv_kernel<true>, dim3((M + PM_ROWS - 1) / PM_ROWS), dim3(PM_NT), PM_LDS, st, x, ln0_g, ln0_b, w1, b1, w2, b2,
                     ln1_g, ln1_b, nullptr, feat, M, eps);
  SF_CHECK_LAUNCH();
  return 0;
}
```

slotformer_amd/csrc/sf_internal.h:

```cpp
#pragma once
#include "../../include/slotformer_hip.h"
#include "sf_common.h"
#include "sf_switches.h"

struct SfThreadOpts {
  int precision = -1;
  int seam = -1;
  int ffn_rows = 0;
  int attn_heads = 0;
  int attn_rows = 0;
  int ffn_tile = 0;
  int layer_tok = 0;
  int cus = 0;
};
SfThreadOpts& sf_thread_opts();
inline int sf_precision(const SfThreadOpts& o) { return o.precision < 0 ? sf_switch(SF_SW_PRECISION) : o.precision; }
inline bool sf_seam_on(const SfThreadOpts& o) { return (o.seam < 0 ? sf_switch(SF_SW_SEAM_FUSED) : o.seam) != 0; }
inline bool sf_layer_tok_on(const SfThreadOpts& o) { return (o.layer_tok == 0 ? sf_switch(SF_SW_LAYER_TOK) : o.layer_tok) > 0; }
inline int sf_ffn_rows(const SfThreadOpts& o) { return o.ffn_rows > 0 ? o.ffn_rows : (sf_switch(SF_SW_FFN_ROWS64) ? 64 : 32); }
int sf_ensure_dyn_lds(const void* kernel, size_t bytes);

int sf_linear_ex(const float* A, SfRowMap amap, const float* W, const float* bias, const float* ln_g,
                 const float* ln_b, float ln_eps, const float* res, SfRowMap rmap, int res_mod,
                 float* C, SfRowMap cmap, int M, int N, int K, int relu, hipStream_t stream, int ln_relu = 0);
int sf_linear_dropout_ex(const float* A, const float* W, const float* bias, const float* res, float* C, int M, int N, int K,
                         int relu, uint32_t drop_seed, uint32_t drop_thresh, float drop_scale, hipStream_t stream);
int sf_layernorm_ex(const float* x, SfRowMap xmap, const float* g, const float* b, float* y, SfRowMap ymap,
                    int rows, int D, float eps, hipStream_t st);
int sf_mha_ex(const float* qkv, float* out, int B, int L, int Lq, int d, int nheads, hipStream_t st);
int sf_lstm_pointwise_ex(const float* gates, const float* c_prev, float* h_out, float* c_out, int R, int H,
                         hipStream_t st);
int sf_sample_dist_ex(const float* dist, const float* noise, SfRowMap nmap, float* out, int R, int D,
                      hipStream_t st);
int sf_copy_rows_ex(const float* src, SfRowMap smap, float* dst, SfRowMap dmap, int rows, int cols,
                    hipStream_t st);
int sf_sa_pick_partials(int HW);
bool sf_pixel_mlp_feat_ok(int C0, int C1);
int sf_pixel_mlp_feat192_ex(const float* x, const float* ln0_g, const float* ln0_b, const void* w1p, const float* b1, const void* w2p,
                            const float* b2, const float* ln1_g, const float* ln1_b, float* feat, int M, float eps, hipStream_t st);
int sf_pixel_mlp_feat_ex(const float* x, const float* ln0_g, const float* ln0_b, const float* w1, const float* b1, const float* w2,
                         const float* b2, const float* ln1_g, const float* ln1_b, float* feat, int M, float eps, hipStream_t st);
bool sf_slot_update_mfma_ok(int D, int H, int P);
struct SfNextStep {
  const float *pm_ln_g, *pm_ln_b;
  const void* pm_w0_p;
  const float* pm_b0;
  const void* pm_w2_p;
  const float* pm_b2;
  int norm_first;
  const void* kd_w_p;
  const float* kd_b;
  const float* noise;
  long long noise_bs;
  float* kdist_out;
  long long kdist_bs;
  float* slots;
};
int sf_slot_update_mfma_ex(const float* part_num, const float* part_den, int P, const float* slots_prev, const void* gru_ih_p,
                           const void* gru_hh_p, const float* gru_b_ih, const float* gru_b_hh, const float* ln_g, const float* ln_b,
                           const void* w1_p, const float* b1, const void* w2_p, const float* b2, float* slots_out, float* out2,
                           long long out2_bs, const float* q_ln_g, const float* q_ln_b, const void* q_w_p, float* q_out, int B, int N,
                           float ln_eps, hipStream_t st, const SfNextStep* next = nullptr, int p_step = 1);
bool sf_slot_attn_sparse_records(const float* k, const float* v, int HW, int D);
bool sf_slot_attn_sparse_records_n(const float* k, const float* v, int HW, int D, int N);
bool sf_slot_update_wide_ok(int D, int H, int P);
int sf_slot_update_wide_ex(const float* part_num, const float* part_den, int P, const float* slots_prev, const void* gru_ih_p, const void* gru_hh_p,
                           const float* gru_b_ih, const float* gru_b_hh, const float* ln_g, const float* ln_b, const void* w1_p, const float* b1,
                           const void* w2_p, const float* b2, float* slots_out, float* out2, long long out2_bs, const float* q_ln_g,
                           const float* q_ln_b, const void* q_w_p, float* q_out, int B, int N, float ln_eps, hipStream_t st);
int sf_slot_update_ex(const float* part_num, const float* part_den, int P, const float* slots_prev,
                      const float* gru_w_ih, const float* gru_w_hh, const float* gru_b_ih, const float* gru_b_hh,
                      const float* ln_g, const float* ln_b, const float* mlp_w1, const float* mlp_b1, const float* mlp_w2,
                      const float* mlp_b2, float* slots_out, float* out2, long long out2_bs, const float* q_ln_g,
                      const float* q_ln_b, const float* q_w, float* q_out, int B, int N, int D, int H, float ln_eps,
                      hipStream_t st);
int sf_slot_prologue_ex(const float* prev, const float* init, const float* pm_ln_g, const float* pm_ln_b, const float* pm_w0_t,
                        const float* pm_b0, const float* pm_w2_t, const float* pm_b2, int norm_first, const float* kd_w_t,
                        const float* kd_b, const float* noise, long long noise_bs, float* kdist_out, long long kdist_bs,
                        const float* q_ln_g, const float* q_ln_b, const float* q_w_t, float* slots_out, float* q_out, int B,
                        int N, int D, float ln_eps, hipStream_t st);
int sf_slot_attn_iter_ex(const float* k, const float* v, int ld, long long batch_stride, const float* q,
                         float* part_num, float* part_den, float* attn_out, long long attn_batch_stride, int B,
                         int HW, int N, int D, float scale, float eps, hipStream_t st);

enum { SF_K_CONV_NHWC = 0, SF_K_CONV_FIRST = 1, SF_K_LINEAR = 2, SF_K_SA_ITER = 3, SF_K_SA_UPDATE = 4,
       SF_K_MHA = 5, SF_K_FFN = 6, SF_K_SEAM = 7, SF_K_DECONV = 8, SF_K_LAYER_TOK = 9, SF_K_NUM = 10 };
void sf_prof_begin(int cls, hipStream_t st, double work);
void sf_prof_end(int cls, hipStream_t st);
void sf_prof_suppress(int on);
int sf_qkv_attn_ex(const float* x, const float* ln_g, const float* ln_b, float ln_eps, const float* in_proj_w,
                   const float* in_proj_b, float* out, int B, int L, int Lq, int d, int nheads, hipStream_t st);
int sf_conv5x5_ws_ex(const float* in, const void* w_frag, const float* bias, const float* add, float* out, int F, int H, int W, int Cin, int Cout, int ks,
                     int relu, int n_workgroups, hipStream_t st);
extern "C" int sf_stream_cus(void* stream);
int sf_dbg(const char* key);
extern "C" int sf_stream_cus_known(void* stream);
int sf_conv5x5_rows4_ex(const float* in, const void* w_frag, const float* bias, const float* add, float* out, int F, int H, int W,
                        int Cin, int Cout, int ks, int relu, hipStream_t st);
int sf_conv5x5_rows4_ohwi_ex(const float* in, const float* w_ohwi, void* w_frag, const float* bias, const float* add, float* out, int F, int H,
                             int W, int Cin, int Cout, int ks, int relu, hipStream_t st);
struct SfSlateGenWs {
  float *mem, *memkv[16], *cache[16], *x, *xn, *att, *qc, *x2, *x3, *hid, *lg;
  size_t bytes;
};
SfSlateGenWs sf_slate_gen_carve(void* ws, const sf_slate_decoder* m, int B, int steps, size_t cache_w, bool chain);
int sf_deconv5x5s2_ex(const float* in, const void* w_frag, const float* bias, const float* head_w, const float* head_b, float* out, int R,
                      int H, int W, int Cin, int Cout, int ks, int stride, int relu, hipStream_t st);
int sf_conv5x5_rows4_head_ex(const float* in, const void* w_frag, const float* bias, const float* head_w, const float* head_b, float* dec,
                             int F, int H, int W, int Cin, int Cout, int ks, hipStream_t st);
int sf_conv5x5_halo_ex(const float* in, const float* w_packed, const float* bias, const float* add, float* out, int F,
                       int H, int W, int Cin, int Cout, int ks, int relu, hipStream_t st);
int sf_pixel_mlp_kv_ex(const float* x, const float* ln0_g, const float* ln0_b, const float* w1, const float* b1,
                       const float* w2, const float* b2, const float* ln1_g, const float* ln1_b, const float* wkv,
                       float* kv, int M, int C0, int C1, int ND, float eps, hipStream_t st);

bool sf_layer_fused_ok(int d, int heads, int ffn, int L);
int sf_conv_first_grouped_ex(const float* img, long long frame_stride, int fgroup, long long group_stride, const float* w, const float* bias,
                             const float* add, float* out, int F, int Cin, int Hin, int Win, int Cout, int ks, int stride, int relu, hipStream_t st);
int sf_conv_first_ex(const float* img, long long frame_stride, const float* w, const float* bias, const float* add,
                     float* out, int F, int Cin, int Hin, int Win, int Cout, int ks, int stride, int relu, hipStream_t st);
```

slotformer_amd/csrc/slot_chain.h:

```cpp
#pragma once
#include "sf_internal.h"

struct SfChainWeights {
  const void *gru_ih_p, *gru_hh_p;
  const float *gru_b_ih, *gru_b_hh, *ln_g, *ln_b;
  const void* w1_p;
  const float* b1;
  const void* w2_p;
  const float* b2;
  const float *q_ln_g, *q_ln_b;
  const void* q_w_p;
  const float *pm_ln_g, *pm_ln_b;
  const void* pm_w0_p;
  const float* pm_b0;
  const void* pm_w2_p;
  const float* pm_b2;
  int pm_norm_first;
  const void* kd_w_p;
  const float* kd_b;
};

bool sf_slot_chain_ok(int D, int H, int HW, int N);
int sf_slot_chain_ex(const void* feat_planes, int NB, int B, int T, int HW, int N, int iters, float scale, float eps, float ln_eps, float* slotsA, float* slotsB,
                     float* lat, float* q, float* post, long long post_bs, float* attn, const float* noise, float* kdist, const SfChainWeights* w,
                     hipStream_t st);
bool sf_slot_attn_planes_ok(int HW, int D, int N);
int sf_slot_attn_planes_ex(const void* planes, long long batch_stride_rows, const float* q, float* part_num, float* part_den, float* attn_out,
                           long long attn_batch_stride, int B, int HW, int N, float scale, float eps, hipStream_t st);
int sf_pixel_mlp_feat_planes_ex(const float* x, const float* ln0_g, const float* ln0_b, const float* w1, const float* b1, const float* w2,
                                const float* b2, const float* ln1_g, const float* ln1_b, void* planes, int M, float eps, hipStream_t st);
```

slotformer_amd/engine.py:

```python
import ctypes as C
import os

import torch

from . import _lib
from ._call import ptr, require_device, scratch, stream
from ._lib import lib, check, sf_tfm_layer, sf_rollouter, sf_savi_encoder, sf_savi_decoder
from . import ops, plans

_WORKSPACES = {}


def workspace(device, nbytes, slot=0):
    key = (device.type, device.index, slot)
    cur = _WORKSPACES.get(key)
    if cur is None or cur.numel() < nbytes:
        cur = torch.empty(int(nbytes), dtype=torch.uint8, device=device)
        _WORKSPACES[key] = cur
    return cur


def workspace_for(device, slot, query, *args, at_least=0):
    key = (device.type, device.index, slot)
    ws = _WORKSPACES[key] = scratch(query, *args, device=device, reuse=_WORKSPACES.get(key), at_least=at_least)
# ... 142 lines not shown

def burn_in_of(r):
    return 1 if hasattr(r, 'cond_len') else r.history_len


def rollout(r, slots_all, n_in, pred_len, ws_slot=0, opts=None):
    _require_inference(r, slots_all)
    ops._chk(slots_all)
    if n_in != burn_in_of(r):
        raise RuntimeError(f'slotformer_amd: burn-in of {n_in} frames, but this rollouter consumes {burn_in_of(r)} '
                           '(history_len; 1 for SingleStepSlotRollouter)')
    plan = rollouter_plan(r)
    B, T_total = slots_all.shape[:2]
    ws = workspace_for(slots_all.device, ('roll', ws_slot), lib().sf_rollout_workspace_bytes, C.byref(plan.struct), B)
    o = rollout_opts(opts)
    check(lib().sf_rollout_opts_f32(C.byref(plan.struct), slots_all.data_ptr(), B, T_total, pred_len, ws.data_ptr(),
                                    ws.numel(), stream(), None if o is None else C.byref(o)))
    return slots_all


def rollout_phases(r, slots_all, obs, pred_len, frame_offset, ws_slot=0, opts=None):
    if slots_all.dim() != 4:
        raise ValueError(f'slotformer_amd: rollout slots are [B, T_total, N, C], got {tuple(slots_all.shape)}')
    f, obs, pred_len, hist = int(frame_offset), int(obs), int(pred_len), burn_in_of(r)
    B, T_total = slots_all.shape[:2]
    if f < 1:
        raise ValueError(f'slotformer_amd: frame_offset >= 1, got {frame_offset!r}')
    if f > 1 and hasattr(r, 'cond_len'):
        raise ValueError('slotformer_amd: a SingleStepSlotRollouter rolls out at frame_offset 1 only')
    if B < 1 or pred_len < 0:
        raise ValueError(f'slotformer_amd: rollout of {B} videos for {pred_len} frames')
    if obs < hist * f:
        raise ValueError(f'slotformer_amd: {obs} observed frames, but a burn-in of {hist} frames at frame_offset {f} needs {hist * f}')
    steps = -(-pred_len // f)
    if T_total < obs + steps * f:
        raise ValueError(f'slotformer_amd: every phase runs {steps} steps and frames {obs} .. {obs + steps * f - 1} are written, but the buffer has '
                         f'{T_total} frames (pad it to obs + ceil(pred_len / frame_offset) * frame_offset and slice)')
    _require_inference(r, slots_all)
    ops._chk(slots_all)
    plan = rollouter_plan(r)
    ws = workspace_for(slots_all.device, ('roll', ws_slot), lib().sf_rollout_phases_workspace_bytes, C.byref(plan.struct), B, f)
    o = rollout_opts(opts)
    check(lib().sf_rollout_phases_f32(C.byref(plan.struct), slots_all.data_ptr(), B, T_total, obs, f, pred_len, ws.data_ptr(), ws.numel(),
                                      stream(), None if o is None else C.byref(o)))
    return slots_all


def encoder_plan(m):
    return plans.cached(m, 'encoder', plans.signature(m), _encoder_plan, m)


def _encoder_plan(m):
    plan = plans.Plan()
    s = sf_savi_encoder()
    if m.resolution[0] != m.resolution[1] or m.resolution[0] not in (64, 128):
        raise NotImplementedError(f'resolution {m.resolution}: the encoder needs 64x64 or 128x128 input '
                                  '(visual_resolution is fixed to 64x64, savi.py:226)')
    s.resolution = m.resolution[0]
    ch = list(m.enc_channels)
    n = len(ch) - 1
    if n > 8:
        raise NotImplementedError('at most 8 encoder convs')
    s.enc_layers, s.enc_ks = n, m.enc_ks
    for i, c in enumerate(ch):
        s.enc_channels[i] = c
    for i in range(n):
        conv = m.encoder[i][0]
        w = conv.weight.detach().float().contiguous()
        wp = w if i == 0 else ops.pack_conv_weight(w)
        s.conv_w[i] = plan.dp(wp)
        s.conv_b[i] = plan.dp(conv.bias)
        if i > 0 and w.is_cuda and tuple(w.shape) == (64, 64, 5, 5):
            frag = ops.pack_conv_frag(wp)
            plan.keep.append(frag)
            s.conv_w_frag[i] = frag.data_ptr()
    pe = m.encoder_pos_embedding
    s.pos_table = plan.dp(ops.pos_embed_table(pe.grid.detach().float(), pe.dense.weight.detach().float().contiguous(),
                                              pe.dense.bias.detach().float().contiguous()))
    eo = m.encoder_out_layer
    s.enc_ln_g, s.enc_ln_b = plan.dp(eo[0].weight), plan.dp(eo[0].bias)
    s.enc_fc1_w, s.enc_fc1_b = plan.dp(eo[1].weight), plan.dp(eo[1].bias)
    s.enc_fc2_w, s.enc_fc2_b = plan.dp(eo[3].weight), plan.dp(eo[3].bias)
    s.enc_out_channels = m.enc_out_channels
    s.num_slots, s.slot_size, s.slot_mlp_size = m.num_slots, m.slot_size, m.slot_mlp_size
    s.num_iterations = m.num_iterations
    sa = m.slot_attention
    s.sa_norm_in_g, s.sa_norm_in_b = plan.dp(sa.norm_inputs.weight), plan.dp(sa.norm_inputs.bias)
    s.sa_q_ln_g, s.sa_q_ln_b = plan.dp(sa.project_q[0].weight), plan.dp(sa.project_q[0].bias)
    s.sa_q_w = plan.dp(sa.project_q[1].weight)
    s.sa_q_w_t = plan.dp(sa.project_q[1].weight.detach().float().t().contiguous())
    s.sa_kv_w = plan.dp(torch.cat([sa.project_k.weight.detach(), sa.project_v.weight.detach()], 0).contiguous())
    tr = lambda w: w.detach().float().t().contiguous()
    s.gru_w_ih, s.gru_w_hh = plan.dp(tr(sa.gru.weight_ih)), plan.dp(tr(sa.gru.weight_hh))
    s.gru_b_ih, s.gru_b_hh = plan.dp(sa.gru.bias_ih), plan.dp(sa.gru.bias_hh)
    s.mlp_ln_g, s.mlp_ln_b = plan.dp(sa.mlp[0].weight), plan.dp(sa.mlp[0].bias)
    s.mlp_w1, s.mlp_b1 = plan.dp(tr(sa.mlp[1].weight)), plan.dp(sa.mlp[1].bias)
    s.mlp_w2, s.mlp_b2 = plan.dp(tr(sa.mlp[3].weight)), plan.dp(sa.mlp[3].bias)
    if (m.slot_size, m.slot_mlp_size) in ((128, 256), (192, 384)) and sa.gru.weight_ih.is_cuda:
        s.sa_gru_ih_p, s.sa_gru_hh_p = plan.packed(sa.gru.weight_ih), plan.packed(sa.gru.weight_hh)
        s.sa_mlp_w1_p, s.sa_mlp_w2_p = plan.packed(sa.mlp[1].weight), plan.packed(sa.mlp[3].weight)
        s.sa_q_w_p = plan.packed(sa.project_q[1].weight)
    if m.slot_size == m.enc_out_channels and m.slot_size in (128, 192) and sa.project_k.bias is None and sa.project_v.bias is None:
        wk, wv = sa.project_k.weight.detach().double(), sa.project_v.weight.detach().double()
        mq = (wk.t() @ sa.project_q[1].weight.detach().double()).float().contiguous()
        gih = (sa.gru.weight_ih.detach().double() @ wv).float().contiguous()
        s.sa_fold_q_w, s.sa_fold_q_w_t, s.sa_fold_gru_ih_t = plan.dp(mq), plan.dp(mq.t().contiguous()), plan.dp(gih.t().contiguous())
        if mq.is_cuda and m.slot_size == 192 and ch[-1] == 64:
            s.enc_fc1_p, s.enc_fc2_p = plan.packed(eo[1].weight), plan.packed(eo[3].weight)
        if mq.is_cuda and (m.slot_size, m.slot_mlp_size) in ((128, 256), (192, 384)):
            s.sa_fold_q_w_p, s.sa_fold_gru_ih_p = plan.packed(mq), plan.packed(gih)
    s.init_latents = plan.dp(m.init_latents.detach()[0])
    s.sa_eps = float(sa.eps)
    kd = getattr(m, 'kernel_dist_layer', None)
    if kd is None:
        s.kd_mode = 0
    elif len(kd) == 1:
        s.kd_mode = 1
        s.kd_w0, s.kd_b0 = plan.dp(kd[0].weight), plan.dp(kd[0].bias)
        s.kd_w0_t = plan.dp(tr(kd[0].weight))
    else:
        s.kd_mode = 2
        s.kd_w0, s.kd_b0 = plan.dp(kd[0].weight), plan.dp(kd[0].bias)
        s.kd_ln_g, s.kd_ln_b = plan.dp(kd[1].weight), plan.dp(kd[1].bias)
        s.kd_w3, s.kd_b3 = plan.dp(kd[3].weight), plan.dp(kd[3].bias)
    pred = m.predictor
    rnn = hasattr(pred, 'rnn')
    base = pred.base_predictor if rnn else pred
    s.pred_rnn = int(rnn)
    s.pred_norm_first = int(base.norm_first)
    if hasattr(base, 'transformer_encoder'):
        s.pred_type = 1
        s.pred_num_layers, s.pred_num_heads, s.pred_ffn_dim = base.num_layers, base.num_heads, base.ffn_dim
        s.pred_layers = C.cast(_tfm_layers(plan, base.transformer_encoder), C.POINTER(sf_tfm_layer))
    else:
        s.pred_type = 0
        s.pred_ffn_dim = 2 * m.slot_size
        s.pm_ln_g, s.pm_ln_b = plan.dp(base.ln.weight), plan.dp(base.ln.bias)
        s.pm_w0, s.pm_b0 = plan.dp(base.mlp[0].weight), plan.dp(base.mlp[0].bias)
        s.pm_w2, s.pm_b2 = plan.dp(base.mlp[2].weight), plan.dp(base.mlp[2].bias)
        s.pm_w0_t, s.pm_w2_t = plan.dp(tr(base.mlp[0].weight)), plan.dp(tr(base.mlp[2].weight))
        if s.sa_mlp_w1_p and s.kd_mode == 1 and not rnn and base.mlp[0].weight.is_cuda and tuple(base.mlp[0].weight.shape) == (256, 128):
            s.pm_w0_p, s.pm_w2_p, s.kd_w0_p = plan.packed(base.mlp[0].weight), plan.packed(base.mlp[2].weight), plan.packed(kd[0].weight)
    if rnn:
        s.pred_hidden = pred.hidden_size
        s.lstm_w_ih, s.lstm_w_hh = plan.dp(pred.rnn.weight_ih_l0), plan.dp(pred.rnn.weight_hh_l0)
        s.lstm_b_ih, s.lstm_b_hh = plan.dp(pred.rnn.bias_ih_l0), plan.dp(pred.rnn.bias_hh_l0)
        s.proj_w, s.proj_b = plan.dp(pred.out_projector.weight), plan.dp(pred.out_projector.bias)
    if s.pred_type == 1 and base.norm_first and base.num_heads == 4 and m.init_latents.is_cuda:
        mats = []
        for layer in base.transformer_encoder.layers:
            mats += [layer.self_attn.in_proj_weight, layer.self_attn.out_proj.weight, layer.linear1.weight, layer.linear2.weight]
        if rnn:
            mats += [pred.rnn.weight_ih_l0, pred.rnn.weight_hh_l0, pred.out_projector.weight]
        if all(w.shape[0] % 32 == 0 and w.shape[1] % 16 == 0 for w in mats):
            arr = (C.c_void_p * len(mats))(*[plan.packed(w) for w in mats])
            plan.keep.append(arr)
            s.pred_packed = C.cast(arr, C.POINTER(C.c_void_p))
    plan.struct = s
    return plan


_FORK_STREAMS = {}


def _auto_side_stream(dev):
    if os.environ.get('SF_ENCODE_FORK', '1') == '0' or torch.cuda.is_current_stream_capturing():
# ... 197 lines not shown
```

slotformer_amd/ops.py:

```python
import torch

from ._call import ptr, require_device, scratch, stream
from ._lib import lib, check


def _chk(*ts):
    for t in ts:
        if t is None:
            continue
        if not (torch.is_tensor(t) and t.is_cuda and t.dtype == torch.float32 and t.is_contiguous()):
            raise RuntimeError('slotformer_amd ops need contiguous float32 tensors on a HIP device '
                               f'(got {type(t).__name__} {getattr(t, "dtype", None)} '
                               f'{getattr(t, "device", None)}); there is no CPU fallback')


def linear(x, weight, bias=None, ln=None, residual=None, relu=False, ln_eps=1e-5):
    _chk(x, weight, bias, residual, *(ln or ()))
    K = x.shape[-1]
    N = weight.shape[0]
    M = x.numel() // K
    out = torch.empty(*x.shape[:-1], N, device=x.device, dtype=torch.float32)
    g, b = (ln if ln is not None else (None, None))
    check(lib().sf_linear_f32(ptr(x), K, ptr(weight), ptr(bias), ptr(g), ptr(b), ln_eps, ptr(residual), N, ptr(out), N,
                              M, N, K, int(relu), stream()))
# ... 39 lines not shown
    return out


def deconv5x5s2_head(x, w_frag, bias, head_w, head_b):
    _chk(x, bias, head_w, head_b)
    R, H, W, _ = x.shape
    dec = torch.empty(R, 4 * H * W, 4, device=x.device, dtype=torch.float32)
    check(lib().sf_deconv5x5s2_head_frag_f32(ptr(x), w_frag.data_ptr(), ptr(bias), ptr(head_w), ptr(head_b), ptr(dec), R, H, W, stream()))
    return dec


def conv5x5_frag(x, w_frag, bias, relu=True, add=None):
    _chk(x, bias, add)
    F_, H, W, Cin = x.shape
    out = torch.empty(F_, H, W, 64, device=x.device, dtype=torch.float32)
    check(lib().sf_conv5x5_frag_f32(ptr(x), w_frag.data_ptr(), ptr(bias), ptr(add), ptr(out), F_, H, W, int(relu), stream()))
    return out


def conv5x5_ws(x, w_frag, bias, relu=True, add=None, n_workgroups=0):
    _chk(x, bias, add)
    F_, H, W, Cin = x.shape
    out = torch.empty(F_, H, W, 64, device=x.device, dtype=torch.float32)
    check(lib().sf_conv5x5_ws_f32(ptr(x), w_frag.data_ptr(), ptr(bias), ptr(add), ptr(out), F_, H, W, int(relu), int(n_workgroups), stream()))
    return out


def pack_deconv_weight(w):
    _chk(w)
    out = torch.empty(w.shape[1], w.shape[2], w.shape[3], w.shape[0], device=w.device, dtype=torch.float32)
    check(lib().sf_pack_deconv_weight_f32(ptr(w), ptr(out), w.shape[0], w.shape[1], w.shape[2], stream()))
    return out


def conv_transpose2d_nhwc(x, w_packed, bias, stride, relu=True):
    _chk(x, w_packed, bias)
    F_, H, W, Cin = x.shape
    Cout, ks = w_packed.shape[0], w_packed.shape[1]
    out = torch.empty(F_, H * stride, W * stride, Cout, device=x.device, dtype=torch.float32)
    check(lib().sf_conv_transpose2d_nhwc_f32(ptr(x), ptr(w_packed), ptr(bias), ptr(out), F_, H, W, Cin, Cout, ks, stride,
                                             int(relu), stream()))
    return out


def pos_embed_table(grid, dense_w, dense_b):
    grid = grid.reshape(-1, 4).contiguous()
    _chk(grid, dense_w, dense_b)
    out = torch.empty(grid.shape[0], dense_w.shape[0], device=grid.device, dtype=torch.float32)
    check(lib().sf_pos_embed_table_f32(ptr(grid), ptr(dense_w), ptr(dense_b), ptr(out), grid.shape[0],
                                       dense_w.shape[0], stream()))
    return out


def conv2d_first(img, weight, bias, stride, relu=True, add=None):
    _chk(img, weight, bias, add)
    F_, Cin, H, W = img.shape
    Cout, ks = weight.shape[0], weight.shape[2]
    Ho = (H + 2 * (ks // 2) - ks) // stride + 1
    Wo = (W + 2 * (ks // 2) - ks) // stride + 1
    out = torch.empty(F_, Ho, Wo, Cout, device=img.device, dtype=torch.float32)
    check(lib().sf_conv2d_nchw_in_f32(ptr(img), Cin * H * W, ptr(weight), ptr(bias), ptr(add), ptr(out), F_, Cin, H, W,
                                      Cout, ks, stride, int(relu), stream()))
    return out


def conv2d_first_clip(clip, weight, bias, stride, relu=True, add=None):
    _chk(clip, weight, bias, add)
    B, T, Cin, H, W = clip.shape
    Cout, ks = weight.shape[0], weight.shape[2]
    Ho = (H + 2 * (ks // 2) - ks) // stride + 1
    Wo = (W + 2 * (ks // 2) - ks) // stride + 1
    out = torch.empty(T * B, Ho, Wo, Cout, device=clip.device, dtype=torch.float32)
    check(lib().sf_conv2d_nchw_in_grouped_f32(ptr(clip), T * Cin * H * W, B, Cin * H * W, ptr(weight), ptr(bias), ptr(add), ptr(out), T * B, Cin,
                                              H, W, Cout, ks, stride, int(relu), stream()))
    return out


def pixel_feat(x, ln0, fc1, fc2, ln1, form=3, eps=1e-5):
    _chk(x, *ln0, *fc1, *fc2, *ln1)
    M = x.shape[0]
    out = torch.empty(M, 256, device=x.device, dtype=torch.bfloat16) if form == 4 else torch.empty(M, 128, device=x.device, dtype=torch.float32)
    check(lib().sf_pixel_feat_f32(ptr(x), ptr(ln0[0]), ptr(ln0[1]), ptr(fc1[0]), ptr(fc1[1]), ptr(fc2[0]), ptr(fc2[1]), ptr(ln1[0]), ptr(ln1[1]),
                                  out.data_ptr(), M, eps, form, stream()))
    return out


def conv2d_nhwc(x, w_packed, bias, relu=True, add=None):
    _chk(x, w_packed, bias, add)
    F_, H, W, Cin = x.shape
    Cout, ks = w_packed.shape[0], w_packed.shape[1]
    out = torch.empty(F_, H, W, Cout, device=x.device, dtype=torch.float32)
    check(lib().sf_conv2d_nhwc_f32(ptr(x), ptr(w_packed), ptr(bias), ptr(add), ptr(out), F_, H, W, Cin, Cout, ks,
                                   int(relu), stream()))
    return out


def conv_wgrad(a, x, stride=1, partial=None):
    _chk(a, x, partial)
    F_, H, W, CA = a.shape
    _, Hx, Wx, _ = x.shape
    if partial is None:
        partial = torch.empty(lib().sf_conv_wgrad_partial_floats(CA, 5), device=a.device, dtype=torch.float32)
    out = torch.empty(CA, 64, 5, 5, device=a.device, dtype=torch.float32)
    check(lib().sf_conv_wgrad_f32(ptr(a), CA, F_, H, W, ptr(x), Hx, Wx, int(stride), 5, F_ * H * W, ptr(out), ptr(partial), partial.numel(), stream()))
    return out


def pack_conv_bwd_weight(w):
    _chk(w)
    out = torch.empty(w.shape[1], w.shape[2], w.shape[3], w.shape[0], device=w.device, dtype=torch.float32)
    check(lib().sf_pack_conv_bwd_weight_f32(ptr(w), ptr(out), w.shape[0], w.shape[1], w.shape[2], stream()))
    return out


def conv2d_nhwc_bwd_data(g, w_packed, stride=1, relu_mask=None):
    _chk(g, w_packed, relu_mask)
    F_, H, W, Cin = g.shape
    Cout, ks = w_packed.shape[0], w_packed.shape[1]
    out = torch.empty(F_, H // stride, W // stride, Cout, device=g.device, dtype=torch.float32)
    check(lib().sf_conv2d_nhwc_bwd_data_f32(ptr(g), ptr(w_packed), ptr(relu_mask), ptr(out), F_, H, W, Cin, Cout, ks, int(stride), stream()))
    return out


def conv_first_wgrad(img, dy, frame_stride=None):
    _chk(img, dy)
    F_, res = img.shape[0], img.shape[-1]
    ws = scratch(lib().sf_conv_first_wgrad_workspace_bytes, F_, device=img.device, at_least=16)
    out = torch.empty(64, 3, 5, 5, device=img.device, dtype=torch.float32)
    check(lib().sf_conv_first_wgrad_f32(ptr(img), int(frame_stride or 3 * res * res), res, ptr(dy), F_, ptr(out), ws.data_ptr(), ws.numel(),
                                        stream()))
    return out


def pos_dense_grad(d, grid):
    _chk(d, grid)
    F_, HW, C_ = d.shape
    dw, db = torch.empty(C_, 4, device=d.device), torch.empty(C_, device=d.device)
    dtab = torch.empty(HW, C_, device=d.device)
    check(lib().sf_pos_dense_grad_f32(ptr(d), F_, HW, C_, ptr(grid), ptr(dw), ptr(db), ptr(dtab), stream()))
    return dw, db, dtab


def savi_decode_head_bwd(dec, d_recon, act, out_w, want_param_grads=True):
    _chk(dec, d_recon, act, out_w)
    F_, N, HW, _ = dec.shape
    Cl = out_w.shape[1]
    d_dec, d_act = torch.empty_like(dec), torch.empty_like(act)
    gw = torch.empty(4, Cl, device=dec.device) if want_param_grads else None
    gb = torch.empty(4, device=dec.device) if want_param_grads else None
    ws = scratch(lib().sf_savi_decode_head_bwd_workspace_bytes, Cl, device=dec.device, at_least=16)
    check(lib().sf_savi_decode_head_bwd_f32(ptr(dec), ptr(d_recon), ptr(act), ptr(out_w), ptr(d_dec), ptr(d_act), ptr(gw), ptr(gb), F_, N, HW, Cl,
                                            ws.data_ptr(), ws.numel(), stream()))
    return d_dec, d_act, gw, gb


def slot_attn_iter(k, v, q, eps=1e-6, want_attn=False):
    _chk(k, v, q)
    B, HW, D = k.shape
    N = q.shape[1]
    P = lib().sf_slot_attn_num_partials(HW)
    pn = torch.empty(B, P, N, D, device=k.device, dtype=torch.float32)
    pd = torch.empty(B, P, N, device=k.device, dtype=torch.float32)
    attn = torch.empty(B, N, HW, device=k.device, dtype=torch.float32) if want_attn else None
    check(lib().sf_slot_attn_iter_f32(ptr(k), ptr(v), D, HW * D, ptr(q), ptr(pn), ptr(pd), ptr(attn), B, HW, N, D,
                                      float(D)**-0.5, eps, stream()))
    return pn, pd, attn
# ... 842 lines not shown
```

Measured before the change: 704,200.

## Move position-table add into pixel MLP kernel and prepack its bf16 weight fragments

Result: no change. 710,900 (median of 6 runs) (+1.0%).

```diff
diff --git a/include/slotformer_hip.h b/include/slotformer_hip.h
--- a/include/slotformer_hip.h
+++ b/include/slotformer_hip.h
@@ -40,6 +40,11 @@
 int sf_pack_conv_weight_f32(const float* w_oihw, float* w_ohwi, int Cout, int Cin, int ks, void* stream);
 int sf_pixel_feat_f32(const float* x, const float* ln0_g, const float* ln0_b, const float* w1, const float* b1, const float* w2,
                       const float* b2, const float* ln1_g, const float* ln1_b, float* feat, int M, float eps, int form, void* stream);
+int sf_pixel_feat_pos_f32(const float* x, const float* pos, int HW, const float* ln0_g, const float* ln0_b, const float* w1, const float* b1,
+                          const float* w2, const float* b2, const float* ln1_g, const float* ln1_b, const void* packed, void* feat, int M, float eps,
+                          int planes, void* stream);
+size_t sf_pixel_feat_packed_bytes(void);
+int sf_pack_pixel_feat_weights(const float* w1, const float* w2, void* packed, void* stream);
 size_t sf_conv_frag_bytes(int Cout, int Cin, int ks);
 int sf_set_conv_fp16x2(int on);
 int sf_get_conv_fp16x2(void);
@@ -598,6 +603,8 @@
   const void *enc_fc1_p, *enc_fc2_p;
   const void* conv_w_frag[8];
   const void *pm_w0_p, *pm_w2_p, *kd_w0_p;
+  const void* enc_fc_frag;
+  int enc_pos_in_conv;
 } sf_savi_encoder;
 
 size_t sf_savi_encode_workspace_bytes(const sf_savi_encoder* m, int B);
diff --git a/slotformer_amd/_lib.py b/slotformer_amd/_lib.py
--- a/slotformer_amd/_lib.py
+++ b/slotformer_amd/_lib.py
@@ -122,7 +122,7 @@
          ('sa_gru_ih_p', C.c_void_p), ('sa_gru_hh_p', C.c_void_p), ('sa_mlp_w1_p', C.c_void_p), ('sa_mlp_w2_p', C.c_void_p),
          ('sa_q_w_p', C.c_void_p), ('sa_fold_q_w', FP), ('sa_fold_q_w_t', FP), ('sa_fold_gru_ih_t', FP), ('sa_fold_q_w_p', C.c_void_p),
          ('sa_fold_gru_ih_p', C.c_void_p), ('pred_packed', C.POINTER(C.c_void_p)), ('enc_fc1_p', C.c_void_p), ('enc_fc2_p', C.c_void_p),
-         ('conv_w_frag', C.c_void_p * 8), ('pm_w0_p', C.c_void_p), ('pm_w2_p', C.c_void_p), ('kd_w0_p', C.c_void_p)])
+         ('conv_w_frag', C.c_void_p * 8), ('pm_w0_p', C.c_void_p), ('pm_w2_p', C.c_void_p), ('kd_w0_p', C.c_void_p), ('enc_fc_frag', C.c_void_p), ('enc_pos_in_conv', C.c_int)])
 
 
 class sf_slate_block(C.Structure):
@@ -178,6 +178,9 @@
     'sf_conv2d_nhwc_f32': (I, [FP, FP, FP, FP, FP, I, I, I, I, I, I, I, VP]),
     'sf_pack_conv_weight_f32': (I, [FP, FP, I, I, I, VP]),
     'sf_pixel_feat_f32': (I, [FP] * 10 + [I, F32, I, VP]),
+    'sf_pixel_feat_pos_f32': (I, [FP, FP, I] + [FP] * 8 + [VP, VP, I, F32, I, VP]),
+    'sf_pixel_feat_packed_bytes': (SZ, []),
+    'sf_pack_pixel_feat_weights': (I, [FP, FP, VP, VP]),
     'sf_conv_frag_bytes': (SZ, [I, I, I]),
     'sf_set_conv_fp16x2': (I, [I]),
     'sf_get_conv_fp16x2': (I, []),
diff --git a/slotformer_amd/csrc/engine.hip b/slotformer_amd/csrc/engine.hip
--- a/slotformer_amd/csrc/engine.hip
+++ b/slotformer_amd/csrc/engine.hip
@@ -540,6 +540,7 @@
   int KV = 2;
   int n_pre = 0;
   bool batched = false;
+  bool pos_at_pixel = false;
   enum Feat { KV_GEMMS, KV_FUSED, FOLD_ROWS, FOLD_192, FOLD_PLANES } feat = KV_GEMMS;
   const float *q_w = nullptr, *q_w_t = nullptr, *gru_ih_t = nullptr;
   const void *q_w_p = nullptr, *gru_ih_p = nullptr;
@@ -635,16 +636,17 @@
   p.chain = p.batched && p.chain_model && sf_switch(SF_SW_SLOT_CHAIN);
   if (p.chain && ws_bytes < enc_ws_bytes(m, B, T, p)) p.chain = false;
   if (p.batched && ws_bytes < enc_ws_bytes(m, B, T, p)) p.batched = false;
+  p.pos_at_pixel = p.batched && (p.feat == EncodePlan::FOLD_PLANES || p.feat == EncodePlan::FOLD_ROWS) && sf_switch(SF_SW_PIXEL_TOK) && !m->enc_pos_in_conv;
   return p;
 }
 
 int run_cnn_layers(const sf_savi_encoder* m, const float* src, long long frame_stride, int nb, float* dst, float* featA, float* featB,
-                   int i0, int i1, hipStream_t st) {
+                   int i0, int i1, hipStream_t st, bool add_pos = true) {
   const int res = m->resolution;
   for (int i = i0; i < i1; ++i) {
     const bool lastc = (i == m->enc_layers - 1);
     const int cin = m->enc_channels[i], cout = m->enc_channels[i + 1];
-    const float* add = lastc ? m->pos_table : nullptr;
+    const float* add = lastc && add_pos ? m->pos_table : nullptr;
     float* out = lastc ? dst : ((i & 1) ? featB : featA);
     const float* cur = i == 0 ? nullptr : (((i - 1) & 1) ? featB : featA);
     if (i == 0) {
@@ -664,7 +666,7 @@
   return 0;
 }
 
-int enc_cnn_all_steps(const sf_savi_encoder* m, const float* img, int B, int T, float* const* big, hipStream_t st) {
+int enc_cnn_all_steps(const sf_savi_encoder* m, const float* img, int B, int T, float* const* big, hipStream_t st, bool add_pos) {
   const int res = m->resolution, c1 = m->enc_channels[1];
   const long long frame_elems = (long long)3 * res * res;
   const int rc = sf_conv_first_grouped_ex(img, (long long)T * frame_elems, B, frame_elems, m->conv_w[0], m->conv_b[0], nullptr, big[0], B * T,
@@ -673,13 +675,16 @@
   for (int t = 0; t < T && rc == 1; ++t)
     SF_TRY(sf_conv2d_nchw_in_f32(img + (long long)t * frame_elems, (long long)T * frame_elems, m->conv_w[0], m->conv_b[0], nullptr,
                                  big[0] + (long long)t * B * ENC_HW * c1, B, m->enc_channels[0], res, res, c1, m->enc_ks, res == 128 ? 2 : 1, 1, st));
-  return run_cnn_layers(m, nullptr, 0, B * T, big[2], big[0], big[1], 1, m->enc_layers, st);
-}
-
-int enc_feature_planes(const sf_savi_encoder* m, const float* img, int B, int T, float* const* big, void* planes, hipStream_t st) {
-  SF_TRY(enc_cnn_all_steps(m, img, B, T, big, st));
+  return run_cnn_layers(m, nullptr, 0, B * T, big[2], big[0], big[1], 1, m->enc_layers, st, add_pos);
+}
+
+SfPixelExtra enc_pixel_extra(const sf_savi_encoder* m, bool pos_at_pixel) {
+  return SfPixelExtra{pos_at_pixel ? m->pos_table : nullptr, ENC_HW, m->enc_fc_frag};
+}
+int enc_feature_planes(const sf_savi_encoder* m, const float* img, int B, int T, float* const* big, void* planes, hipStream_t st, bool pos_at_pixel) {
+  SF_TRY(enc_cnn_all_steps(m, img, B, T, big, st, !pos_at_pixel));
   return sf_pixel_mlp_feat_planes_ex(big[2], m->enc_ln_g, m->enc_ln_b, m->enc_fc1_w, m->enc_fc1_b, m->enc_fc2_w, m->enc_fc2_b, m->sa_norm_in_g, m->sa_norm_in_b,
-                                     planes, B * T * ENC_HW, 1e-5f, st);
+                                     planes, B * T * ENC_HW, 1e-5f, st, enc_pixel_extra(m, pos_at_pixel));
 }
 int enc_slots_chain(const sf_savi_encoder* m, const void* planes, const float* noise, const float* prev, float* post, long long post_bs, float* kernel_dist,
                     float* attn, int NB, int B, int T, const SlotRows& r, hipStream_t st) {
@@ -731,6 +736,7 @@
   const int HW = ENC_HW, B = a.B, Bc = enc_chunk(B), Cl = m->enc_channels[m->enc_layers], Ce = m->enc_out_channels, D = m->slot_size;
   const long long frame_elems = (long long)3 * m->resolution * m->resolution;
   const float ln_eps = 1e-5f;
+  const SfPixelExtra px = enc_pixel_extra(m, p.pos_at_pixel && t >= p.n_pre);
   for (int b0 = 0; b0 < B; b0 += Bc) {
     const int nb = (B - b0 < Bc) ? (B - b0) : Bc, Mp = nb * HW;
     const float* cur;
@@ -749,10 +755,10 @@
                                      m->sa_norm_in_g, m->sa_norm_in_b, kv + (long long)b0 * HW * Ce, Mp, ln_eps, st));
     } else if (p.feat == EncodePlan::FOLD_PLANES) {
       SF_TRY(sf_pixel_mlp_feat_planes_ex(cur, m->enc_ln_g, m->enc_ln_b, m->enc_fc1_w, m->enc_fc1_b, m->enc_fc2_w, m->enc_fc2_b, m->sa_norm_in_g, m->sa_norm_in_b,
-                                         (char*)kv + (size_t)b0 * HW * 512, Mp, ln_eps, st));
+                                         (char*)kv + (size_t)b0 * HW * 512, Mp, ln_eps, st, px));
     } else if (p.feat == EncodePlan::FOLD_ROWS) {
       SF_TRY(sf_pixel_mlp_feat_ex(cur, m->enc_ln_g, m->enc_ln_b, m->enc_fc1_w, m->enc_fc1_b, m->enc_fc2_w, m->enc_fc2_b,
-                                  m->sa_norm_in_g, m->sa_norm_in_b, kv + (long long)b0 * HW * Ce, Mp, ln_eps, st));
+                                  m->sa_norm_in_g, m->sa_norm_in_b, kv + (long long)b0 * HW * Ce, Mp, ln_eps, st, px));
     } else {
       float* kv_dst = kv + (long long)b0 * HW * 2 * D;
       int rc = 1;
@@ -956,7 +962,7 @@
   float* big[3];
   enc_cnn_take(bp, big, 3, m, (size_t)B * T);
   if (!bp.ok) return sf_set_err(-1, "workspace too small", __FILE__, __LINE__);
-  return enc_feature_planes(m, img, B, T, big, planes, (hipStream_t)stream);
+  return enc_feature_planes(m, img, B, T, big, planes, (hipStream_t)stream, plan_encode(m, B, T, 0, false, ~(size_t)0).pos_at_pixel);
 }
 size_t sf_savi_slots_chain_workspace_bytes(const sf_savi_encoder* m, int videos) {
   if (!m || videos <= 0) return 0;
@@ -1032,10 +1038,10 @@
     SF_CHECK_LAUNCH();
   }
   if (p.chain) {
-    SF_TRY(enc_feature_planes(m, img, B, T, w.big, w.planes, st_main));
+    SF_TRY(enc_feature_planes(m, img, B, T, w.big, w.planes, st_main, p.pos_at_pixel));
     return enc_slots_chain(m, w.planes, noise, prev, post_slots, (long long)T * N * D, kernel_dist, attn, 1, B, T, w.rows, st_main);
   }
-  if (p.batched) SF_TRY(enc_cnn_all_steps(m, img, B, T, w.big, st_main));
+  if (p.batched) SF_TRY(enc_cnn_all_steps(m, img, B, T, w.big, st_main, !p.pos_at_pixel));
   bool next_done = false;
   for (int t = 0; t < T; ++t) {
     float* kv = w.kv + (size_t)(t % p.KV) * B * ENC_HW * 2 * D;
diff --git a/slotformer_amd/csrc/pixel_mlp.hip b/slotformer_amd/csrc/pixel_mlp.hip
--- a/slotformer_amd/csrc/pixel_mlp.hip
+++ b/slotformer_amd/csrc/pixel_mlp.hip
@@ -219,17 +219,18 @@
 bool sf_pixel_mlp_feat_ok(int C0, int C1) { return C0 == PM_C0 && C1 == PM_C1; }
 template <bool PLANES>
 static int sf_pixel_feat_tok_launch(const float* x, const float* ln0_g, const float* ln0_b, const float* w1, const float* b1, const float* w2, const float* b2,
-                                    const float* ln1_g, const float* ln1_b, void* out, int M, float eps, hipStream_t st);
+                                    const float* ln1_g, const float* ln1_b, void* out, int M, float eps, hipStream_t st, const SfPixelExtra& e);
 
 static int sf_pixel_feat_stream_launch(const float* x, const float* ln0_g, const float* ln0_b, const float* w1, const float* b1, const float* w2,
                                        const float* b2, const float* ln1_g, const float* ln1_b, float* feat, int M, float eps, hipStream_t st,
                                        int tile = 0);
 
 int sf_pixel_mlp_feat_ex(const float* x, const float* ln0_g, const float* ln0_b, const float* w1, const float* b1, const float* w2,
-                         const float* b2, const float* ln1_g, const float* ln1_b, float* feat, int M, float eps, hipStream_t st) {
+                         const float* b2, const float* ln1_g, const float* ln1_b, float* feat, int M, float eps, hipStream_t st, const SfPixelExtra& e) {
   if (M <= 0) return 0;
   constexpr int stream = 1;
-  if (sf_switch(SF_SW_PIXEL_TOK)) return sf_pixel_feat_tok_launch<false>(x, ln0_g, ln0_b, w1, b1, w2, b2, ln1_g, ln1_b, feat, M, eps, st);
+  if (sf_switch(SF_SW_PIXEL_TOK)) return sf_pixel_feat_tok_launch<false>(x, ln0_g, ln0_b, w1, b1, w2, b2, ln1_g, ln1_b, feat, M, eps, st, e);
+  SF_REQUIRE(!e.pos, "pixel chain: the position table is added by the pixel-stationary form only");
   if (stream) return sf_pixel_feat_stream_launch(x, ln0_g, ln0_b, w1, b1, w2, b2, ln1_g, ln1_b, feat, M, eps, st);
   SF_TRY(sf_ensure_dyn_lds((const void*)pixel_mlp_kv_kernel<true>, (size_t)(PM_LDS)));
   sf_prof_begin(SF_K_LINEAR, st, 2.0 * M * (double)(PM_C0 * PM_C1 + PM_C1 * PM_C1));
@@ -614,45 +615,79 @@
 constexpr size_t PT_LDS = (size_t)PT_VEC + PV_N * 4;
 }
 
-template <bool PLANES>
-__global__ __launch_bounds__(PT_NT) void pixel_feat_tok_kernel(const float* __restrict__ x, const float* __restrict__ ln0_g, const float* __restrict__ ln0_b,
+__device__ __forceinline__ void pt_build_fragments(const float* __restrict__ w1, const float* __restrict__ w2, int t, char* dst0) {
+  f32x4 wa[6], wb[6];
+#pragma unroll
+  for (int it = 0; it < 6; ++it) {
+    const int f = t + it * PT_NT, fl = f & 63, fi = fl & 31, fh = fl >> 5, fr = f >> 6;
+    const float* p;
+    int second;
+    if (fr < 16) {
+      const int blk = fr >> 2, ks = fr & 3;
+      p = w1 + (long long)(32 * blk + fi) * PM_C0 + 32 * fh + 8 * ks;
+      second = 4;
+    } else {
+      const int g2 = fr - 16, ob = g2 >> 3, blk = (g2 >> 1) & 3, sx = g2 & 1;
+      const int orow = 64 * ((fi >> 2) & 1) + 16 * ob + 4 * (fi >> 3) + (fi & 3);
+      p = w2 + (long long)orow * PM_C1 + 32 * blk + 16 * sx + 4 * fh;
+      second = 8;
+    }
+    wa[it] = *(const f32x4*)p;
+    wb[it] = *(const f32x4*)(p + second);
+  }
+#pragma unroll
+  for (int it = 0; it < 6; ++it) {
+    const int f = t + it * PT_NT, fl = f & 63, fr = f >> 6;
+    const bf16x4 ah = __builtin_convertvector(wa[it], bf16x4), bh = __builtin_convertvector(wb[it], bf16x4);
+    const bf16x4 al = __builtin_convertvector(wa[it] - __builtin_convertvector(ah, f32x4), bf16x4);
+    const bf16x4 bl = __builtin_convertvector(wb[it] - __builtin_convertvector(bh, f32x4), bf16x4);
+    char* dst = dst0 + (size_t)fr * 2048 + fl * 16;
+    *(bf16x8*)dst = __builtin_shufflevector(ah, bh, 0, 1, 2, 3, 4, 5, 6, 7);
+    *(bf16x8*)(dst + 1024) = __builtin_shufflevector(al, bl, 0, 1, 2, 3, 4, 5, 6, 7);
+  }
+}
+
+__global__ __launch_bounds__(PT_NT) void pixel_feat_pack_kernel(const float* __restrict__ w1, const float* __restrict__ w2, char* __restrict__ packed) {
+  pt_build_fragments(w1, w2, threadIdx.x, packed);
+}
+
+template <bool PLANES, bool POS>
+__global__ __launch_bounds__(PT_NT) void pixel_feat_tok_kernel(const float* __restrict__ x, const float* __restrict__ pos, int HW,
+                                                               const float* __restrict__ ln0_g, const float* __restrict__ ln0_b,
                                                                const float* __restrict__ w1, const float* __restrict__ b1, const float* __restrict__ w2,
                                                                const float* __restrict__ b2, const float* __restrict__ ln1_g, const float* __restrict__ ln1_b,
-                                                               void* __restrict__ out, int M, float eps, int tpw) {
+                                                               const uint4* __restrict__ packed, void* __restrict__ out, int M, float eps, int tpw) {
   extern __shared__ __attribute__((aligned(16))) char pt_lds[];
   const int t = threadIdx.x, lane = t & 63;
   const int wave = __builtin_amdgcn_readfirstlane(t >> 6);
   const int n = lane & 31, h = lane >> 5;
-  {
-    f32x4 wa[6], wb[6];
-#pragma unroll
-    for (int it = 0; it < 6; ++it) {
-      const int f = t + it * PT_NT, fl = f & 63, fi = fl & 31, fh = fl >> 5, fr = f >> 6;
-      const float* p;
-      int second;
-      if (fr < 16) {
-        const int blk = fr >> 2, ks = fr & 3;
-        p = w1 + (long long)(32 * blk + fi) * PM_C0 + 32 * fh + 8 * ks;
-        second = 4;
-      } else {
-        const int g2 = fr - 16, ob = g2 >> 3, blk = (g2 >> 1) & 3, sx = g2 & 1;
-        const int orow = 64 * ((fi >> 2) & 1) + 16 * ob + 4 * (fi >> 3) + (fi & 3);
-        p = w2 + (long long)orow * PM_C1 + 32 * blk + 16 * sx + 4 * fh;
-        second = 8;
-      }
-      wa[it] = *(const f32x4*)p;
-      wb[it] = *(const f32x4*)(p + second);
-    }
-#pragma unroll
-    for (int it = 0; it < 6; ++it) {
-      const int f = t + it * PT_NT, fl = f & 63, fr = f >> 6;
-      const bf16x4 ah = __builtin_convertvector(wa[it], bf16x4), bh = __builtin_convertvector(wb[it], bf16x4);
-      const bf16x4 al = __builtin_convertvector(wa[it] - __builtin_convertvector(ah, f32x4), bf16x4);
-      const bf16x4 bl = __builtin_convertvector(wb[it] - __builtin_convertvector(bh, f32x4), bf16x4);
-      char* dst = pt_lds + (size_t)fr * 2048 + fl * 16;
-      *(bf16x8*)dst = __builtin_shufflevector(ah, bh, 0, 1, 2, 3, 4, 5, 6, 7);
-      *(bf16x8*)(dst + 1024) = __builtin_shufflevector(al, bl, 0, 1, 2, 3, 4, 5, 6, 7);
-    }
+  const long long ntile = ((long long)M + 31) / 32, tstep = (long long)gridDim.x * (PT_NT / 64);
+  long long tile = (long long)blockIdx.x * (PT_NT / 64) + wave;
+  auto row_of = [&](long long tl) {
+    const long long px = tl * 32 + n;
+    return px < M ? (int)px : M - 1;
+  };
+  f32x4 xn[8], pn[POS ? 8 : 1];
+  auto request = [&](long long tl) __attribute__((always_inline)) {
+    const int r = row_of(tl);
+    const float* xr = x + (long long)r * PM_C0 + 32 * h;
+#pragma unroll
+    for (int i = 0; i < 8; ++i) xn[i] = *(const f32x4*)(xr + 4 * i);
+    if constexpr (POS) {
+      const float* pr = pos + (unsigned)((r % HW) * PM_C0 + 32 * h);
+#pragma unroll
+      for (int i = 0; i < 8; ++i) pn[i] = *(const f32x4*)(pr + 4 * i);
+    }
+  };
+  if (tile < ntile) request(tile);
+  if (packed) {
+    uint4 wv[PT_VEC / 16 / PT_NT];
+#pragma unroll
+    for (int it = 0; it < PT_VEC / 16 / PT_NT; ++it) wv[it] = packed[t + it * PT_NT];
+#pragma unroll
+    for (int it = 0; it < PT_VEC / 16 / PT_NT; ++it) *(uint4*)(pt_lds + (size_t)(t + it * PT_NT) * 16) = wv[it];
+  } else {
+    pt_build_fragments(w1, w2, t, pt_lds);
   }
   float* PV = (float*)(pt_lds + PT_VEC);
   for (int i = t; i < PV_N; i += PT_NT)
@@ -668,31 +703,21 @@
     return h ? o + v : v + o;
   };
   const char* wl = pt_lds + lane * 16;
-  const long long ntile = ((long long)M + 31) / 32, tstep = (long long)gridDim.x * (PT_NT / 64);
-  long long tile = (long long)blockIdx.x * (PT_NT / 64) + wave;
-  auto row_of = [&](long long tl) {
-    const long long px = tl * 32 + n;
-    return px < M ? px : (long long)M - 1;
-  };
-  f32x4 xn[8];
-  if (tile < ntile) {
-    const float* xr = x + row_of(tile) * PM_C0 + 32 * h;
-#pragma unroll
-    for (int i = 0; i < 8; ++i) xn[i] = *(const f32x4*)(xr + 4 * i);
-  }
+  int pv4 = PT_VEC / 4 + 4 * h, pv32 = PT_VEC / 4 + 32 * h, pv64 = PT_VEC / 4 + 64 * h;
+  asm volatile("" : "+v"(pv4), "+v"(pv32), "+v"(pv64));
+  const float* L = (const float*)pt_lds;
 #pragma unroll 1
   for (int ti = 0; ti < tpw; ++ti, tile += tstep) {
     if (tile >= ntile) break;
     const long long p0 = tile * 32;
-    const long long pix = row_of(tile);
+    const int pix = row_of(tile);
     f32x4 xv[8];
 #pragma unroll
-    for (int i = 0; i < 8; ++i) xv[i] = xn[i];
-    if (tile + tstep < ntile) {
-      const float* xr = x + row_of(tile + tstep) * PM_C0 + 32 * h;
-#pragma unroll
-      for (int i = 0; i < 8; ++i) xn[i] = *(const f32x4*)(xr + 4 * i);
-    }
+    for (int i = 0; i < 8; ++i) {
+      if constexpr (POS) xv[i] = xn[i] + pn[i];
+      else xv[i] = xn[i];
+    }
+    if (tile + tstep < ntile) request(tile + tstep);
     float s0 = 0.f;
 #pragma unroll
     for (int i = 0; i < 8; ++i) s0 += (xv[i][0] + xv[i][1]) + (xv[i][2] + xv[i][3]);
@@ -707,9 +732,9 @@
     bf16x8 xh[4], xl[4];
 #pragma unroll
     for (int ks = 0; ks < 4; ++ks) {
-      const int c = 32 * h + 8 * ks;
-      sf_split8(xv[2 * ks] * rstd * *(const f32x4*)(PV + PV_G0 + c) + *(const f32x4*)(PV + PV_B0 + c),
-                xv[2 * ks + 1] * rstd * *(const f32x4*)(PV + PV_G0 + c + 4) + *(const f32x4*)(PV + PV_B0 + c + 4), xh[ks], xl[ks]);
+      const int c = 8 * ks;
+      sf_split8(xv[2 * ks] * rstd * *(const f32x4*)(L + pv32 + PV_G0 + c) + *(const f32x4*)(L + pv32 + PV_B0 + c),
+                xv[2 * ks + 1] * rstd * *(const f32x4*)(L + pv32 + PV_G0 + c + 4) + *(const f32x4*)(L + pv32 + PV_B0 + c + 4), xh[ks], xl[ks]);
     }
     bf16x8 hh[8], hl[8];
 #pragma unroll
@@ -743,7 +768,7 @@
 #pragma unroll
           for (int gg = 0; gg < 2; ++gg) {
             const int g = 2 * sx + gg;
-            const f32x4 bb = *(const f32x4*)(PV + PV_B1 + 32 * blk + 8 * g + 4 * h);
+            const f32x4 bb = *(const f32x4*)(L + pv4 + PV_B1 + 32 * blk + 8 * g);
 #pragma unroll
             for (int q = 0; q < 4; ++q) u[gg][q] = fmaxf(acc[e][4 * g + q] + bb[q], 0.f);
           }
@@ -779,7 +804,7 @@
     for (int ob = 0; ob < 4; ++ob)
 #pragma unroll
       for (int g = 0; g < 4; ++g) {
-        const f32x4 bb = *(const f32x4*)(PV + PV_B2 + 64 * h + 16 * ob + 4 * g);
+        const f32x4 bb = *(const f32x4*)(L + pv64 + PV_B2 + 16 * ob + 4 * g);
 #pragma unroll
         for (int q = 0; q < 4; ++q) {
           Y[ob][4 * g + q] += bb[q];
@@ -804,8 +829,8 @@
         f32x4 y[2];
 #pragma unroll
         for (int gg = 0; gg < 2; ++gg) {
-          const int g = 2 * gp + gg, c = 64 * h + 16 * ob + 4 * g;
-          const f32x4 ga = *(const f32x4*)(PV + PV_G1 + c), be = *(const f32x4*)(PV + PV_BE1 + c);
+          const int g = 2 * gp + gg, c = 16 * ob + 4 * g;
+          const f32x4 ga = *(const f32x4*)(L + pv64 + PV_G1 + c), be = *(const f32x4*)(L + pv64 + PV_BE1 + c);
 #pragma unroll
           for (int q = 0; q < 4; ++q) y[gg][q] = Y[ob][4 * g + q] * rstd1 * ga[q] + be[q];
         }
@@ -814,11 +839,11 @@
           if constexpr (PLANES) {
             bf16x8 yh, yl;
             sf_split8(y[0], y[1], yh, yl);
-            __bf16* pr = (__bf16*)out + pix * (2 * PM_C1);
+            __bf16* pr = (__bf16*)out + (long long)pix * (2 * PM_C1);
             *(bf16x8*)(pr + c0) = yh;
             *(bf16x8*)(pr + PM_C1 + c0) = yl;
           } else {
-            float* pr = (float*)out + pix * PM_C1;
+            float* pr = (float*)out + (long long)pix * PM_C1;
             *(f32x4*)(pr + c0) = y[0];
             *(f32x4*)(pr + c0 + 4) = y[1];
           }
@@ -827,27 +852,56 @@
   }
 }
 
-template <bool PLANES>
-static int sf_pixel_feat_tok_launch(const float* x, const float* ln0_g, const float* ln0_b, const float* w1, const float* b1, const float* w2, const float* b2,
-                                    const float* ln1_g, const float* ln1_b, void* out, int M, float eps, hipStream_t st) {
+template <bool PLANES, bool POS>
+static int sf_pixel_feat_tok_launch_t(const float* x, const float* ln0_g, const float* ln0_b, const float* w1, const float* b1, const float* w2, const float* b2,
+                                      const float* ln1_g, const float* ln1_b, void* out, int M, float eps, hipStream_t st, const SfPixelExtra& e) {
   static_assert(PT_LDS <= 160 * 1024, "LDS budget");
-  SF_TRY(sf_ensure_dyn_lds((const void*)pixel_feat_tok_kernel<PLANES>, PT_LDS));
+  SF_TRY(sf_ensure_dyn_lds((const void*)pixel_feat_tok_kernel<PLANES, POS>, PT_LDS));
   const long long ntile = ((long long)M + 31) / 32;
   long long grid = (ntile + (PT_NT / 64) - 1) / (PT_NT / 64);
   const int cus = sf_stream_cus((void*)st);
   if (grid > cus) grid = cus;
   const int tpw = (int)((ntile + grid * (PT_NT / 64) - 1) / (grid * (PT_NT / 64)));
   sf_prof_begin(SF_K_LINEAR, st, 2.0 * M * (double)(PM_C0 * PM_C1 + PM_C1 * PM_C1));
-  hipLaunchKernelGGL(pixel_feat_tok_kernel<PLANES>, dim3((unsigned)grid), dim3(PT_NT), PT_LDS, st, x, ln0_g, ln0_b, w1, b1, w2, b2, ln1_g, ln1_b, out, M, eps, tpw);
+  hipLaunchKernelGGL((pixel_feat_tok_kernel<PLANES, POS>), dim3((unsigned)grid), dim3(PT_NT), PT_LDS, st, x, e.pos, e.HW, ln0_g, ln0_b, w1, b1, w2, b2, ln1_g,
+                     ln1_b, (const uint4*)e.packed, out, M, eps, tpw);
   sf_prof_end(SF_K_LINEAR, st);
   SF_CHECK_LAUNCH();
   return 0;
 }
+template <bool PLANES>
+static int sf_pixel_feat_tok_launch(const float* x, const float* ln0_g, const float* ln0_b, const float* w1, const float* b1, const float* w2, const float* b2,
+                                    const float* ln1_g, const float* ln1_b, void* out, int M, float eps, hipStream_t st, const SfPixelExtra& e) {
+  SF_REQUIRE(!e.pos || (e.HW > 0 && e.HW <= (1 << 24)), "pixel chain: a position table needs its row count (at most 2^24)");
+  if (e.pos) return sf_pixel_feat_tok_launch_t<PLANES, true>(x, ln0_g, ln0_b, w1, b1, w2, b2, ln1_g, ln1_b, out, M, eps, st, e);
+  return sf_pixel_feat_tok_launch_t<PLANES, false>(x, ln0_g, ln0_b, w1, b1, w2, b2, ln1_g, ln1_b, out, M, eps, st, e);
+}
 
 int sf_pixel_mlp_feat_planes_ex(const float* x, const float* ln0_g, const float* ln0_b, const float* w1, const float* b1, const float* w2,
-                                const float* b2, const float* ln1_g, const float* ln1_b, void* planes, int M, float eps, hipStream_t st) {
-  if (sf_switch(SF_SW_PIXEL_TOK)) return sf_pixel_feat_tok_launch<true>(x, ln0_g, ln0_b, w1, b1, w2, b2, ln1_g, ln1_b, planes, M, eps, st);
+                                const float* b2, const float* ln1_g, const float* ln1_b, void* planes, int M, float eps, hipStream_t st,
+                                const SfPixelExtra& e) {
+  if (sf_switch(SF_SW_PIXEL_TOK)) return sf_pixel_feat_tok_launch<true>(x, ln0_g, ln0_b, w1, b1, w2, b2, ln1_g, ln1_b, planes, M, eps, st, e);
+  SF_REQUIRE(!e.pos, "pixel chain: the position table is added by the pixel-stationary form only");
   return sf_pixel_feat_stream_launch_t<64, true>(x, ln0_g, ln0_b, w1, b1, w2, b2, ln1_g, ln1_b, (float*)planes, M, eps, st);
+}
+
+extern "C" size_t sf_pixel_feat_packed_bytes(void) { return PT_VEC; }
+extern "C" int sf_pack_pixel_feat_weights(const float* w1, const float* w2, void* packed, void* stream) {
+  SF_REQUIRE(w1 && w2 && packed, "sf_pack_pixel_feat_weights: null pointer");
+  hipLaunchKernelGGL(pixel_feat_pack_kernel, dim3(1), dim3(PT_NT), 0, (hipStream_t)stream, w1, w2, (char*)packed);
+  SF_CHECK_LAUNCH();
+  return 0;
+}
+
+extern "C" int sf_pixel_feat_pos_f32(const float* x, const float* pos, int HW, const float* ln0_g, const float* ln0_b, const float* w1, const float* b1,
+                                     const float* w2, const float* b2, const float* ln1_g, const float* ln1_b, const void* packed, void* feat, int M,
+                                     float eps, int planes, void* stream) {
+  SF_REQUIRE(x && ln0_g && ln0_b && w1 && b1 && w2 && b2 && ln1_g && ln1_b && feat && M > 0, "sf_pixel_feat_pos_f32: null pointer / empty problem");
+  SF_REQUIRE(!pos || HW > 0, "sf_pixel_feat_pos_f32: a position table needs HW > 0");
+  SF_REQUIRE(sf_get_precision() == 1, "sf_pixel_feat_pos_f32: split-bf16 mode only");
+  const SfPixelExtra e{pos, HW, packed};
+  if (planes) return sf_pixel_feat_tok_launch<true>(x, ln0_g, ln0_b, w1, b1, w2, b2, ln1_g, ln1_b, feat, M, eps, (hipStream_t)stream, e);
+  return sf_pixel_feat_tok_launch<false>(x, ln0_g, ln0_b, w1, b1, w2, b2, ln1_g, ln1_b, feat, M, eps, (hipStream_t)stream, e);
 }
 
 extern "C" int sf_pixel_feat_f32(const float* x, const float* ln0_g, const float* ln0_b, const float* w1, const float* b1, const float* w2,
@@ -857,7 +911,7 @@
   SF_REQUIRE(sf_get_precision() == 1, "sf_pixel_feat_f32: split-bf16 mode only");
   hipStream_t st = (hipStream_t)stream;
   if (form == 4) return sf_pixel_mlp_feat_planes_ex(x, ln0_g, ln0_b, w1, b1, w2, b2, ln1_g, ln1_b, feat, M, eps, st);
-  if (form == 3) return sf_pixel_feat_tok_launch<false>(x, ln0_g, ln0_b, w1, b1, w2, b2, ln1_g, ln1_b, feat, M, eps, st);
+  if (form == 3) return sf_pixel_feat_tok_launch<false>(x, ln0_g, ln0_b, w1, b1, w2, b2, ln1_g, ln1_b, feat, M, eps, st, SfPixelExtra{});
   if (form >= 1) return sf_pixel_feat_stream_launch(x, ln0_g, ln0_b, w1, b1, w2, b2, ln1_g, ln1_b, feat, M, eps, st, form == 1 ? 128 : 64);
   SF_TRY(sf_ensure_dyn_lds((const void*)pixel_mlp_kv_kernel<true>, (size_t)(PM_LDS)));
   hipLaunchKernelGGL(pixel_mlp_kv_kernel<true>, dim3((M + PM_ROWS - 1) / PM_ROWS), dim3(PM_NT), PM_LDS, st, x, ln0_g, ln0_b, w1, b1, w2, b2,
diff --git a/slotformer_amd/csrc/sf_internal.h b/slotformer_amd/csrc/sf_internal.h
--- a/slotformer_amd/csrc/sf_internal.h
+++ b/slotformer_amd/csrc/sf_internal.h
@@ -38,8 +38,14 @@
 bool sf_pixel_mlp_feat_ok(int C0, int C1);
 int sf_pixel_mlp_feat192_ex(const float* x, const float* ln0_g, const float* ln0_b, const void* w1p, const float* b1, const void* w2p,
                             const float* b2, const float* ln1_g, const float* ln1_b, float* feat, int M, float eps, hipStream_t st);
+struct SfPixelExtra {
+  const float* pos = nullptr;
+  int HW = 0;
+  const void* packed = nullptr;
+};
 int sf_pixel_mlp_feat_ex(const float* x, const float* ln0_g, const float* ln0_b, const float* w1, const float* b1, const float* w2,
-                         const float* b2, const float* ln1_g, const float* ln1_b, float* feat, int M, float eps, hipStream_t st);
+                         const float* b2, const float* ln1_g, const float* ln1_b, float* feat, int M, float eps, hipStream_t st,
+                         const SfPixelExtra& e = SfPixelExtra{});
 bool sf_slot_update_mfma_ok(int D, int H, int P);
 struct SfNextStep {
   const float *pm_ln_g, *pm_ln_b;
diff --git a/slotformer_amd/csrc/slot_chain.h b/slotformer_amd/csrc/slot_chain.h
--- a/slotformer_amd/csrc/slot_chain.h
+++ b/slotformer_amd/csrc/slot_chain.h
@@ -28,4 +28,5 @@
 int sf_slot_attn_planes_ex(const void* planes, long long batch_stride_rows, const float* q, float* part_num, float* part_den, float* attn_out,
                            long long attn_batch_stride, int B, int HW, int N, float scale, float eps, hipStream_t st);
 int sf_pixel_mlp_feat_planes_ex(const float* x, const float* ln0_g, const float* ln0_b, const float* w1, const float* b1, const float* w2,
-                                const float* b2, const float* ln1_g, const float* ln1_b, void* planes, int M, float eps, hipStream_t st);
+                                const float* b2, const float* ln1_g, const float* ln1_b, void* planes, int M, float eps, hipStream_t st,
+                                const SfPixelExtra& e = SfPixelExtra{});
diff --git a/slotformer_amd/engine.py b/slotformer_amd/engine.py
--- a/slotformer_amd/engine.py
+++ b/slotformer_amd/engine.py
@@ -248,6 +248,10 @@
     s.enc_fc1_w, s.enc_fc1_b = plan.dp(eo[1].weight), plan.dp(eo[1].bias)
     s.enc_fc2_w, s.enc_fc2_b = plan.dp(eo[3].weight), plan.dp(eo[3].bias)
     s.enc_out_channels = m.enc_out_channels
+    if eo[1].weight.is_cuda and tuple(eo[1].weight.shape) == (128, 64) and tuple(eo[3].weight.shape) == (128, 128):
+        frag = ops.pack_pixel_feat(plan.f32(eo[1].weight), plan.f32(eo[3].weight))
+        plan.keep.append(frag)
+        s.enc_fc_frag = frag.data_ptr()
     s.num_slots, s.slot_size, s.slot_mlp_size = m.num_slots, m.slot_size, m.slot_mlp_size
     s.num_iterations = m.num_iterations
     sa = m.slot_attention
diff --git a/slotformer_amd/ops.py b/slotformer_amd/ops.py
--- a/slotformer_amd/ops.py
+++ b/slotformer_amd/ops.py
@@ -145,6 +145,23 @@
     out = torch.empty(M, 256, device=x.device, dtype=torch.bfloat16) if form == 4 else torch.empty(M, 128, device=x.device, dtype=torch.float32)
     check(lib().sf_pixel_feat_f32(ptr(x), ptr(ln0[0]), ptr(ln0[1]), ptr(fc1[0]), ptr(fc1[1]), ptr(fc2[0]), ptr(fc2[1]), ptr(ln1[0]), ptr(ln1[1]),
                                   out.data_ptr(), M, eps, form, stream()))
+    return out
+
+
+def pack_pixel_feat(w1, w2):
+    _chk(w1, w2)
+    out = torch.empty(lib().sf_pixel_feat_packed_bytes(), device=w1.device, dtype=torch.uint8)
+    check(lib().sf_pack_pixel_feat_weights(ptr(w1), ptr(w2), out.data_ptr(), stream()))
+    return out
+
+
+def pixel_feat_pos(x, ln0, fc1, fc2, ln1, pos=None, packed=None, planes=False, eps=1e-5):
+    _chk(x, *ln0, *fc1, *fc2, *ln1, pos)
+    M = x.shape[0]
+    out = torch.empty(M, 256, device=x.device, dtype=torch.bfloat16) if planes else torch.empty(M, 128, device=x.device, dtype=torch.float32)
+    check(lib().sf_pixel_feat_pos_f32(ptr(x), ptr(pos), 0 if pos is None else pos.shape[0], ptr(ln0[0]), ptr(ln0[1]), ptr(fc1[0]), ptr(fc1[1]),
+                                      ptr(fc2[0]), ptr(fc2[1]), ptr(ln1[0]), ptr(ln1[1]), None if packed is None else packed.data_ptr(),
+                                      out.data_ptr(), M, eps, int(planes), stream()))
     return out
 
 
```
